# tensorlink-lab/tensorlink

Hardware: AMD Instinct MI355X
Metric: output tokens/sec (Qwen2.5-7B serving, PP sharded) (higher is better)
Workload: dtype bf16; 1 GPU; model=Qwen/Qwen2.5-7B-Instruct, global_batch=256, seq_len=512, parallelism=pp1, micro_batches=4

## Files before the change

### tensorlink_amd/models/dense.py

```python

from __future__ import annotations

import dataclasses

import math
from typing import List, Optional

import torch
import torch.nn as nn

from tensorlink_amd import ops
from tensorlink_amd.models.configs import ModelConfig


class KVCache:

    def __init__(self, n_layers: int, batch: int, max_seq: int, config,
                 device, dtype=torch.bfloat16):
        self.k = [torch.zeros(batch, config.num_key_value_heads, max_seq,
                              config.head_dim, device=device, dtype=dtype)
                  for _ in range(n_layers)]
        self.v = [torch.zeros_like(self.k[0]) for _ in range(n_layers)]
        self.seq_lens = torch.zeros(batch, device=device, dtype=torch.int32)
        self.max_seq = max_seq
        self.batch = batch

    def reset(self):
        self.seq_lens.zero_()

    def append(self, layer: int, k_new: torch.Tensor, v_new: torch.Tensor,
               positions: torch.Tensor):
        B, S_new, Hkv, D = k_new.shape
        idx = positions.to(self.k[layer].device, torch.long)
        idx = idx.view(B, 1, S_new, 1).expand(B, Hkv, S_new, D)
        self.k[layer].scatter_(2, idx, k_new.transpose(1, 2))
        self.v[layer].scatter_(2, idx, v_new.transpose(1, 2))

    def advance(self, n: int):
        self.seq_lens += n


class TLLinear(nn.Linear):

    def forward(self, x):
        return ops.linear(x, self.weight, self.bias)


def compute_inv_freq(config: ModelConfig) -> torch.Tensor:
    D = config.head_dim
    inv = 1.0 / (config.rope_theta ** (
        torch.arange(0, D, 2, dtype=torch.float32) / D))
    rs = config.rope_scaling
    if rs and rs.get("rope_type", rs.get("type")) == "llama3":
        factor = rs["factor"]
        lo, hi = rs["low_freq_factor"], rs["high_freq_factor"]
        orig = rs["original_max_position_embeddings"]
        wavelen = 2 * math.pi / inv
        smooth = (orig / wavelen - lo) / (hi - lo)
        smoothed = (1 - smooth) / factor * inv + smooth * inv
        inv = torch.where(wavelen > orig / lo, inv / factor, inv)
        mid = (wavelen <= orig / lo) & (wavelen >= orig / hi)
        inv = torch.where(mid, smoothed, inv)
    return inv


class Attention(nn.Module):
    def __init__(self, config: ModelConfig):
        super().__init__()
        self.config = config
        h, q, kv = config.hidden_size, config.q_size, config.kv_size
        bias = config.qkv_bias
        self.qkv_proj = TLLinear(h, q + 2 * kv, bias=bias)
        self.o_proj = TLLinear(q, h, bias=False)
        self.q_size, self.kv_size = q, kv
        self.n_heads = config.num_attention_heads
        self.n_kv = config.num_key_value_heads
        self.head_dim = config.head_dim
        self.scale = 1.0 / math.sqrt(self.head_dim)
        self.use_qk_norm = config.architecture == "qwen3"
        if self.use_qk_norm:
            self.q_norm = nn.Parameter(torch.ones(self.head_dim))
            self.k_norm = nn.Parameter(torch.ones(self.head_dim))
        self.register_buffer("inv_freq", compute_inv_freq(config),
                             persistent=False)

    def _split_qkv(self, qkv, B, S):
        q, k, v = qkv.split([self.q_size, self.kv_size, self.kv_size],
                            dim=-1)
        q = q.reshape(B, S, self.n_heads, self.head_dim)
        k = k.reshape(B, S, self.n_kv, self.head_dim)
        v = v.reshape(B, S, self.n_kv, self.head_dim)
        return q, k, v

    def forward(self, x: torch.Tensor, positions: torch.Tensor,
                kv_cache: Optional[KVCache] = None, layer_idx: int = 0,
                training: bool = False) -> torch.Tensor:
        B, S, H = x.shape
        eps = self.config.rms_norm_eps
        qkv = self.qkv_proj(x)
        flat_pos = positions.reshape(-1)

        if training or kv_cache is None:
            q, k, v = self._split_qkv(qkv, B, S)
            if self.use_qk_norm:
                q = ops.rmsnorm(q.contiguous(), self.q_norm.to(q.dtype), eps)
                k = ops.rmsnorm(k.contiguous(), self.k_norm.to(k.dtype), eps)
            if training:
                q2, k2 = ops.apply_rope(q.reshape(B * S, self.n_heads, -1),
                                        k.reshape(B * S, self.n_kv, -1),
                                        flat_pos, self.inv_freq)
                q = q2.view(B, S, self.n_heads, -1)
                k = k2.view(B, S, self.n_kv, -1)
                out = ops.attention_train(q, k, v, causal=True,
                                          scale=self.scale)
            else:
                q = q.contiguous()
                k = k.contiguous()
                ops.apply_rope_(q.view(B * S, self.n_heads, -1),
                                k.view(B * S, self.n_kv, -1), flat_pos,
                                self.inv_freq)
                out = ops.attention_prefill(q, k, v.contiguous(),
                                            causal=True, scale=self.scale)
            return self.o_proj(out.reshape(B, S, -1))

        table = getattr(kv_cache, "table", None)
        if self.use_qk_norm:
            q, k, v = self._split_qkv(qkv, B, S)
            q = ops.rmsnorm(q.contiguous(), self.q_norm.to(q.dtype), eps)
            k = ops.rmsnorm(k.contiguous(), self.k_norm.to(k.dtype), eps)
            qkv = torch.cat([q.reshape(B, S, -1), k.reshape(B, S, -1),
                             v.reshape(B, S, -1)], dim=-1)
        q = ops.rope_append_(qkv.reshape(B * S, -1), kv_cache.k[layer_idx],
                             kv_cache.v[layer_idx], flat_pos, self.inv_freq,
                             S, self.n_heads, self.n_kv, block_table=table)
        q = q.view(B, S, self.n_heads, self.head_dim)
        if S == 1:
            out = ops.attention_decode(
                q, kv_cache.k[layer_idx], kv_cache.v[layer_idx],
                kv_cache.seq_lens + 1, scale=self.scale, block_table=table)
        else:
            if B > 1:
                assert int(kv_cache.seq_lens.min()) == \
                    int(kv_cache.seq_lens.max()), \
                    "ragged cached prefill needs per-row q_off"
            off = int(kv_cache.seq_lens.max())
            kv_len = off + S
            if table is None:
                k_attn = kv_cache.k[layer_idx][:, :, :kv_len].permute(
                    0, 2, 1, 3).contiguous()
                v_attn = kv_cache.v[layer_idx][:, :, :kv_len].permute(
                    0, 2, 1, 3).contiguous()
            else:
                k_attn, v_attn = kv_cache.gather_contiguous(layer_idx, kv_len)
            out = ops.attention_prefill(q, k_attn, v_attn, causal=True,
                                        scale=self.scale, q_off=off)
        return self.o_proj(out.reshape(B, S, -1))


class MLP(nn.Module):
    def __init__(self, config: ModelConfig):
        super().__init__()
        h, i = config.hidden_size, config.intermediate_size
        self.inter = i
        self.gate_up_proj = TLLinear(h, 2 * i, bias=False)
        self.down_proj = TLLinear(i, h, bias=False)

    def forward(self, x):
        gu = self.gate_up_proj(x)
        if torch.is_grad_enabled() and gu.requires_grad:
            gate, up = gu.split([self.inter, self.inter], dim=-1)
            return self.down_proj(ops.swiglu(gate.contiguous(),
                                             up.contiguous()))
        return self.down_proj(ops.swiglu_fused(gu))


class MoEMLP(nn.Module):

    def __init__(self, config: ModelConfig):
        super().__init__()
        h, i = config.hidden_size, config.intermediate_size
        self.num_experts = config.num_local_experts
        self.top_k = config.num_experts_per_tok
        self.gate = nn.Linear(h, self.num_experts, bias=False)
        expert_cfg = (config if config.expert_intermediate_size == i
                      else dataclasses.replace(
                          config,
                          intermediate_size=config.expert_intermediate_size))
        self.experts = nn.ModuleList([MLP(expert_cfg)
                                      for _ in range(self.num_experts)])

    def _fused_kind(self):
        from tensorlink_amd.models.quant import Fp4Linear, Fp8Linear
        e0 = self.experts[0]
        if isinstance(e0.gate_up_proj, Fp8Linear):
            return "fp8"
        if isinstance(e0.gate_up_proj, Fp4Linear):
            for e in self.experts:
                for p in (e.gate_up_proj, e.down_proj):
                    if not (isinstance(p, Fp4Linear) and p.bias is None
                            and p.out_features % 64 == 0
                            and p.in_features % 128 == 0):
                        return None
            return "fp4"
        if isinstance(e0.gate_up_proj, nn.Linear) \
                and e0.gate_up_proj.bias is None:
            return "bf16"
        return None

    def _tables(self, dev, kind):
        wname = {"fp8": "weight_fp8", "fp4": "packed"}.get(kind, "weight")
        sname = {"fp8": "scale", "fp4": "exponents"}.get(kind)
        gus = [getattr(e.gate_up_proj, wname) for e in self.experts]
        key = (str(dev), kind, gus[0].data_ptr())
        if getattr(self, "_tbl_key", None) != key:
            downs = [getattr(e.down_proj, wname) for e in self.experts]

            def mk(ts):
                if kind == "fp4":
                    assert all(t.is_contiguous()
                               and t.data_ptr() % 16 == 0 for t in ts), \
                        "fp4 expert tensors must be contiguous and " \
                        "16-byte aligned"
                return torch.tensor([t.data_ptr() for t in ts],
                                    dtype=torch.int64, device=dev)
            self._gu_ptrs = mk(gus)
            self._down_ptrs = mk(downs)
            if sname is not None:
                self._gu_scales = mk([getattr(e.gate_up_proj, sname)
                                      for e in self.experts])
                self._down_scales = mk([getattr(e.down_proj, sname)
                                        for e in self.experts])
            else:
                self._gu_scales = self._down_scales = None
            self._tbl_key = key
        return (self._gu_ptrs, self._down_ptrs, self._gu_scales,
                self._down_scales)

    def _fused_forward(self, flat, rw, idx, kind=None):
        C = ops._require_ext()
        kind = kind if kind is not None else self._fused_kind()
        E, k = self.num_experts, self.top_k
        T, H = flat.shape
        P = T * k
        dev = flat.device
        gu_p, down_p, gu_s, down_s = self._tables(dev, kind)
        fi = idx.reshape(-1)
        order = fi.argsort(stable=True)
        counts = torch.zeros(E, device=dev, dtype=torch.long)
        counts.scatter_add_(0, fi, torch.ones_like(fi))
        seg = torch.zeros(E + 1, device=dev, dtype=torch.int32)
        seg[1:] = counts.cumsum(0)
        pair_tok = (order // k).to(torch.int32)
        Ie = self.experts[0].inter
        if kind == "fp4":
            gu = ops.mxfp4_moe_gemm(flat.contiguous(), pair_tok, seg, gu_p,
                                    gu_s, 2 * Ie)
            act = ops.swiglu_fused(gu)
            y_pairs = ops.mxfp4_moe_gemm(act, None, seg, down_p, down_s, H)
        else:
            fp8 = kind == "fp8"
            gu = C.moe_gemm(flat.contiguous(), pair_tok, seg, gu_p, gu_s,
                            2 * Ie, fp8)
            act = ops.swiglu_fused(gu)
            y_pairs = C.moe_gemm(act, None, seg, down_p, down_s, H, fp8)
        y_pairs = y_pairs * rw.reshape(-1)[order].unsqueeze(1)
        inv = torch.empty_like(order)
        inv[order] = torch.arange(P, device=dev, dtype=order.dtype)
        return y_pairs[inv].view(T, k, H).sum(1)

    def forward(self, x):
        B, S, H = x.shape
        flat = x.reshape(-1, H)
        weights, idx = ops.moe_topk_router(self.gate(flat), self.top_k)
        weights = weights.to(x.dtype)
        if (flat.is_cuda and flat.dtype == torch.bfloat16
                and not torch.is_grad_enabled() and ops.extension_loaded()):
            kind = self._fused_kind()
            if kind is not None:
                out = self._fused_forward(flat, weights, idx, kind)
                return out.reshape(B, S, H)
        out = torch.zeros_like(flat)
        for e in range(self.num_experts):
            mask = (idx == e)
            tok, slot = mask.nonzero(as_tuple=True)
            if tok.numel() == 0:
                continue
            out.index_add_(0, tok,
                           self.experts[e](flat[tok]) * weights[tok, slot, None])
        return out.reshape(B, S, H)


class DecoderLayer(nn.Module):
    def __init__(self, config: ModelConfig):
        super().__init__()
        self.config = config
        self.input_layernorm = nn.Parameter(torch.ones(config.hidden_size))
        self.post_attention_layernorm = nn.Parameter(
            torch.ones(config.hidden_size))
        self.self_attn = Attention(config)
        self.mlp = MoEMLP(config) if config.is_moe else MLP(config)

    def forward(self, hidden, positions, kv_cache=None, layer_idx=0,
                training=False):
        eps = self.config.rms_norm_eps
        w_in = self.input_layernorm.to(hidden.dtype)
        w_post = self.post_attention_layernorm.to(hidden.dtype)
        if training or not hidden.is_cuda:
            h = ops.rmsnorm(hidden, w_in, eps)
            hidden = hidden + self.self_attn(h, positions, kv_cache,
                                             layer_idx, training)
            h = ops.rmsnorm(hidden, w_post, eps)
            hidden = hidden + self.mlp(h)
            return hidden
        h = ops.rmsnorm(hidden, w_in, eps)
        attn_out = self.self_attn(h, positions, kv_cache, layer_idx, False)
        h, hidden = ops.rmsnorm_residual(attn_out, hidden, w_post, eps)
        return hidden + self.mlp(h)


class StageModel(nn.Module):

    def __init__(self, config: ModelConfig, layer_start: int, layer_end: int,
                 has_embedding: bool, has_head: bool):
        super().__init__()
        self.config = config
        self.layer_start = layer_start
        self.layer_end = layer_end
        self.has_embedding = has_embedding
        self.has_head = has_head
        if has_embedding:
            self.embed_tokens = nn.Embedding(config.vocab_size,
                                             config.hidden_size)
        self.layers = nn.ModuleList(
            [DecoderLayer(config) for _ in range(layer_end - layer_start)])
        if has_head:
            self.norm = nn.Parameter(torch.ones(config.hidden_size))
            if not (config.tie_word_embeddings and has_embedding):
                self.lm_head = TLLinear(config.hidden_size,
                                        config.vocab_size, bias=False)

    @property
    def num_layers(self):
        return len(self.layers)

    def make_kv_cache(self, batch: int, max_seq: int, device, dtype=None,
                      kv_mode: str = "contiguous"):
        if dtype is None:
            dtype = next(self.parameters()).dtype
        if kv_mode == "paged":
            from tensorlink_amd.models.paged import PagedKVCache
            return PagedKVCache(self.num_layers, batch, max_seq,
                                self.config, device, dtype)
        return KVCache(self.num_layers, batch, max_seq, self.config, device,
                       dtype)

    def embed(self, input_ids: torch.Tensor) -> torch.Tensor:
        w = self.embed_tokens.weight
        return self.embed_tokens(input_ids).to(w.dtype)

    def head(self, hidden: torch.Tensor) -> torch.Tensor:
        h = ops.rmsnorm(hidden, self.norm.to(hidden.dtype),
                        self.config.rms_norm_eps)
        if self.config.tie_word_embeddings and self.has_embedding:
            return h @ self.embed_tokens.weight.t()
        return self.lm_head(h)

    def forward(self, hidden_or_ids, positions, kv_cache: Optional[KVCache]
                = None, training: bool = False,
                return_logits: bool = True) -> torch.Tensor:
        if self.has_embedding and hidden_or_ids.dtype in (torch.int32,
                                                          torch.int64):
            hidden = self.embed(hidden_or_ids)
        else:
            hidden = hidden_or_ids
        ckpt = (training and getattr(self, "grad_checkpointing", False)
                and torch.is_grad_enabled())
        for i, layer in enumerate(self.layers):
            if ckpt:
                hidden = torch.utils.checkpoint.checkpoint(
                    layer, hidden, positions, kv_cache, i, training,
                    use_reentrant=False)
            else:
                hidden = layer(hidden, positions, kv_cache, i, training)
        if kv_cache is not None:
            kv_cache.advance(hidden.shape[1])
        if self.has_head and return_logits:
            return self.head(hidden)
        return hidden


def build_full_model(config: ModelConfig):
    cls = _stage_class(config)
    return cls(config, 0, config.num_hidden_layers, True, True)


def build_stage(config: ModelConfig, spec):
    cls = _stage_class(config)
    return cls(config, spec.layer_start, spec.layer_end,
               spec.has_embedding, spec.has_head)


def _stage_class(config: ModelConfig):
    if config.architecture == "gpt2":
        from tensorlink_amd.models.gpt2 import Gpt2StageModel
        return Gpt2StageModel
    if config.architecture == "neox":
        from tensorlink_amd.models.neox import NeoxStageModel
        return NeoxStageModel
    return StageModel
```

### tensorlink_amd/ops/__init__.py

```python

from __future__ import annotations

import math
from typing import Optional

import torch

from tensorlink_amd.ops import reference as ref

_C = None
_IMPORT_ERROR: Optional[BaseException] = None
try:
    from tensorlink_amd import _C
except Exception as e:
    _IMPORT_ERROR = e


def extension_loaded() -> bool:
    return _C is not None


def _require_ext():
    if _C is None:
        raise RuntimeError(
            "tensorlink_amd._C HIP extension is not built but a CUDA/HIP "
            "tensor reached the op layer. Build it in-tree with "
            "`PYTORCH_ROCM_ARCH=gfx950 python setup.py build_ext --inplace` "
            f"(import error: {_IMPORT_ERROR!r})")
    return _C


def _on_gpu(*tensors: torch.Tensor) -> bool:
    return any(t.is_cuda for t in tensors if isinstance(t, torch.Tensor))


class _RMSNormFn(torch.autograd.Function):
    @staticmethod
    def forward(ctx, x, weight, eps):
        C = _require_ext()
        need_grad = x.requires_grad or weight.requires_grad
        outs = C.rmsnorm_fwd(x.contiguous(), None, weight.contiguous(), eps,
                             need_grad)
        y = outs[0]
        if need_grad:
            ctx.save_for_backward(x, weight, outs[1])
        return y

    @staticmethod
    def backward(ctx, dy):
        C = _require_ext()
        x, weight, rstd = ctx.saved_tensors
        dx, dw = C.rmsnorm_bwd(dy.contiguous(), x.contiguous(),
                               weight.contiguous(), rstd)
        return dx, dw, None


def rmsnorm(x: torch.Tensor, weight: torch.Tensor, eps: float = 1e-6):
    if not _on_gpu(x):
        return ref.rmsnorm(x, weight, eps)
    if torch.is_grad_enabled() and (x.requires_grad or weight.requires_grad):
        return _RMSNormFn.apply(x, weight, eps)
    return _require_ext().rmsnorm_fwd(x.contiguous(), None,
                                      weight.contiguous(), eps, False)[0]


def rmsnorm_residual(x: torch.Tensor, residual: torch.Tensor,
                     weight: torch.Tensor, eps: float = 1e-6):
    if not _on_gpu(x):
        return ref.rmsnorm_residual(x, residual, weight, eps)
    outs = _require_ext().rmsnorm_fwd(x.contiguous(), residual.contiguous(),
                                      weight.contiguous(), eps, False)
    return outs[0], outs[1]


def apply_rope_(q: torch.Tensor, k: torch.Tensor, positions: torch.Tensor,
                inv_freq: torch.Tensor, sign: float = 1.0) -> None:
    if not _on_gpu(q):
        freqs = positions.float()[:, None] * inv_freq.float()[None, :]
        cos, sin = freqs.cos(), freqs.sin()
        qq, kk = ref.apply_rope(q.unsqueeze(0), k.unsqueeze(0), cos,
                                sin * sign)
        q.copy_(qq[0])
        k.copy_(kk[0])
        return
    _require_ext().rope_(q, k, positions.int(), inv_freq.float(), sign)


def rope_append_(qkv: torch.Tensor, k_cache: torch.Tensor,
                 v_cache: torch.Tensor, positions: torch.Tensor,
                 inv_freq: torch.Tensor, S: int, Hq: int, Hkv: int,
                 block_table: Optional[torch.Tensor] = None) -> torch.Tensor:
    if _on_gpu(qkv):
        return _require_ext().rope_append_(
            qkv.contiguous(), k_cache, v_cache, positions.int(),
            inv_freq.float(), S, Hq, Hkv,
            block_table.int() if block_table is not None else None)
    D = k_cache.shape[-1]
    T = qkv.numel() // qkv.shape[-1]
    q = qkv[..., :Hq * D].reshape(T, Hq, D).contiguous()
    k = qkv[..., Hq * D:(Hq + Hkv) * D].reshape(T, Hkv, D).contiguous()
    v = qkv[..., (Hq + Hkv) * D:].reshape(T, Hkv, D).contiguous()
    apply_rope_(q, k, positions, inv_freq)
    B = T // S
    pos = positions.view(B, S).long()
    kB = k.view(B, S, Hkv, D)
    vB = v.view(B, S, Hkv, D)
    if block_table is None:
        for b in range(B):
            k_cache[b, :, pos[b]] = kB[b].transpose(0, 1)
            v_cache[b, :, pos[b]] = vB[b].transpose(0, 1)
    else:
        for b in range(B):
            for s_i in range(S):
                p = int(pos[b, s_i])
                page = int(block_table[b, p // 128])
                k_cache[page, :, p % 128] = kB[b, s_i]
                v_cache[page, :, p % 128] = vB[b, s_i]
    return q


class _RopeFn(torch.autograd.Function):

    @staticmethod
    def forward(ctx, q, k, positions, inv_freq):
        q2, k2 = q.contiguous().clone(), k.contiguous().clone()
        apply_rope_(q2, k2, positions, inv_freq, 1.0)
        ctx.save_for_backward(positions, inv_freq)
        return q2, k2

    @staticmethod
    def backward(ctx, dq, dk):
        positions, inv_freq = ctx.saved_tensors
        dq2, dk2 = dq.contiguous().clone(), dk.contiguous().clone()
        apply_rope_(dq2, dk2, positions, inv_freq, -1.0)
        return dq2, dk2, None, None


def apply_rope(q, k, positions, inv_freq):
    return _RopeFn.apply(q, k, positions, inv_freq)


class _SwiGLUFn(torch.autograd.Function):
    @staticmethod
    def forward(ctx, gate, up):
        C = _require_ext()
        ctx.save_for_backward(gate, up)
        return C.swiglu_fwd(gate.contiguous(), up.contiguous())

    @staticmethod
    def backward(ctx, dout):
        C = _require_ext()
        gate, up = ctx.saved_tensors
        dg, du = C.swiglu_bwd(dout.contiguous(), gate.contiguous(),
                              up.contiguous())
        return dg, du


def swiglu(gate: torch.Tensor, up: torch.Tensor) -> torch.Tensor:
    if not _on_gpu(gate):
        return ref.swiglu(gate, up)
    if torch.is_grad_enabled() and (gate.requires_grad or up.requires_grad):
        return _SwiGLUFn.apply(gate, up)
    return _require_ext().swiglu_fwd(gate.contiguous(), up.contiguous())


def swiglu_fused(gate_up: torch.Tensor) -> torch.Tensor:
    if not _on_gpu(gate_up):
        I = gate_up.shape[-1] // 2
        return ref.swiglu(gate_up[..., :I], gate_up[..., I:])
    return _require_ext().swiglu_fused(gate_up.contiguous())


def attention_prefill(q, k, v, causal: bool = True,
                      scale: Optional[float] = None,
                      q_off: int = 0) -> torch.Tensor:
    scale = scale if scale is not None else 1.0 / math.sqrt(q.shape[-1])
    if not _on_gpu(q):
        return ref.attention_prefill(q, k, v, causal, scale, q_off)
    if (q.shape[1] >= 4096 and q_off == 0 and causal
            and q.shape[1] == k.shape[1]):
        out = torch.nn.functional.scaled_dot_product_attention(
            q.transpose(1, 2), k.transpose(1, 2), v.transpose(1, 2),
            is_causal=True, scale=scale, enable_gqa=True)
        return out.transpose(1, 2)
    return _require_ext().prefill_attn(q.contiguous(), k.contiguous(),
                                       v.contiguous(), scale, causal,
                                       q_off)


class _FlashAttnFn(torch.autograd.Function):

    @staticmethod
    def forward(ctx, q, k, v, causal, scale):
        C = _require_ext()
        out, lse = C.prefill_attn_lse(q.contiguous(), k.contiguous(),
                                      v.contiguous(), scale, causal)
        ctx.save_for_backward(q, k, v, out, lse)
        ctx.causal = causal
        ctx.scale = scale
        return out

    @staticmethod
    def backward(ctx, dout):
        C = _require_ext()
        q, k, v, out, lse = ctx.saved_tensors
        delta = (dout.float() * out.float()).sum(-1)
        delta = delta.permute(0, 2, 1).contiguous()
        dq, dk, dv = C.attn_bwd(q.contiguous(), k.contiguous(),
                                v.contiguous(), dout.contiguous(), lse,
                                delta, ctx.scale, ctx.causal)
        return dq, dk, dv, None, None


def attention_train(q, k, v, causal: bool = True,
                    scale: Optional[float] = None) -> torch.Tensor:
    B, S, Hq, D = q.shape
    Hkv = k.shape[2]
    if scale is None:
        scale = 1.0 / math.sqrt(D)
    if (q.is_cuda and q.dtype == torch.bfloat16 and _C is not None
            and D in (64, 128) and k.shape[1] == S):
        return _FlashAttnFn.apply(q, k, v, causal, scale)
    qt = q.transpose(1, 2)
    kt = k.transpose(1, 2)
    vt = v.transpose(1, 2)
    try:
        out = torch.nn.functional.scaled_dot_product_attention(
            qt, kt, vt, is_causal=causal, scale=scale, enable_gqa=True)
    except (TypeError, RuntimeError):
        rep = Hq // Hkv
        out = torch.nn.functional.scaled_dot_product_attention(
            qt, kt.repeat_interleave(rep, dim=1),
            vt.repeat_interleave(rep, dim=1), is_causal=causal, scale=scale)
    return out.transpose(1, 2)


def attention_decode(q, k_cache, v_cache, seq_lens,
                     scale: Optional[float] = None, n_split: int = 0,
                     block_table: Optional[torch.Tensor] = None
                     ) -> torch.Tensor:
    squeeze = q.dim() == 4
    if squeeze:
        q3 = q.squeeze(1)
    else:
        q3 = q
    scale = scale if scale is not None else 1.0 / math.sqrt(q3.shape[-1])
    if not _on_gpu(q3):
        if block_table is not None:
            B = q3.shape[0]
            L = int(seq_lens.max())
            np_ = (L + 127) // 128
            idx = block_table[:, :np_].long()
            kc = k_cache[idx].permute(0, 1, 3, 2, 4)
            vc = v_cache[idx].permute(0, 1, 3, 2, 4)
            kc = kc.reshape(B, np_ * 128, *kc.shape[3:])[:, :L]
            vc = vc.reshape(B, np_ * 128, *vc.shape[3:])[:, :L]
            out = ref.attention_decode(q3.unsqueeze(1), kc, vc, seq_lens,
                                       scale)
        else:
            out = ref.attention_decode(q3.unsqueeze(1),
                                       k_cache.permute(0, 2, 1, 3),
                                       v_cache.permute(0, 2, 1, 3),
                                       seq_lens, scale)
        return out if squeeze else out.squeeze(1)
    out = _require_ext().decode_attn(
        q3.contiguous(), k_cache, v_cache, seq_lens.int(), scale, n_split,
        block_table.int() if block_table is not None else None)
    return out.unsqueeze(1) if squeeze else out


import os as _os

GEMM_M_MAX = int(_os.environ.get("TL_GEMM_M_MAX", "512"))

gemm_dispatch_count = 0


_LIB_CLASSES = frozenset(
    c for c in _os.environ.get("TL_GEMM_LIB_CLASSES",
                               "gateup").split(",") if c)


def _gemm_class(N: int, K: int) -> str:
    if N >= 65536:
        return "wide"
    if N >= 16384:
        return "gateup"
    if K >= 8192:
        return "deepk"
    return "narrow"


def _use_tl_gemm(M: int, N: int, K: int) -> bool:
    return (K % 32 == 0 and N % 64 == 0 and M <= GEMM_M_MAX
            and _gemm_class(N, K) not in _LIB_CLASSES)


def linear(x: torch.Tensor, weight: torch.Tensor,
           bias: Optional[torch.Tensor] = None) -> torch.Tensor:
    global gemm_dispatch_count
    if (x.is_cuda and not torch.is_grad_enabled()
            and x.dtype == torch.bfloat16
            and not _os.environ.get("TL_NO_SKINNY")):
        K = x.shape[-1]
        M = x.numel() // K
        N = weight.shape[0]
        if _use_tl_gemm(M, N, K):
            gemm_dispatch_count += 1
            return _require_ext().skinny_gemm(
                x.contiguous(), weight,
                bias.to(torch.bfloat16) if bias is not None else None)
    return torch.nn.functional.linear(x, weight, bias)


mxfp4_dispatch_count = 0


def _use_mxfp4_gemm(M: int, N: int, K: int) -> bool:
    return (N > 0 and N % 64 == 0 and K > 0 and K % 128 == 0
            and 1 <= M <= min(GEMM_M_MAX, 512))


def mxfp4_linear(x: torch.Tensor, packed: torch.Tensor,
                 exponents: torch.Tensor,
                 bias: Optional[torch.Tensor] = None) -> torch.Tensor:
    global mxfp4_dispatch_count
    if not _on_gpu(x):
        return ref.mxfp4_linear(x, packed, exponents, bias)
    K = x.shape[-1]
    M = x.numel() // K if K else 0
    N = packed.shape[0]
    if (x.dtype == torch.bfloat16 and _C is not None
            and _use_mxfp4_gemm(M, N, K)):
        mxfp4_dispatch_count += 1
        return _C.mxfp4_gemm(
            x.contiguous(), packed.contiguous(), exponents.contiguous(),
            bias.to(torch.bfloat16).contiguous()
            if bias is not None else None)
    w = ref.dequantize_mxfp4(packed, exponents, dtype=torch.bfloat16)
    return torch.nn.functional.linear(
        x, w.to(x.dtype), bias.to(x.dtype) if bias is not None else None)


mxfp4_moe_dispatch_count = 0


def mxfp4_moe_gemm(x: torch.Tensor, tok_idx: Optional[torch.Tensor],
                   seg_off: torch.Tensor, p_ptrs: torch.Tensor,
                   e_ptrs: torch.Tensor, N: int) -> torch.Tensor:
    global mxfp4_moe_dispatch_count
    out = _require_ext().mxfp4_moe_gemm(x, tok_idx, seg_off, p_ptrs, e_ptrs,
                                        N)
    mxfp4_moe_dispatch_count += 1
    return out


def adamw_(param: torch.Tensor, grad: torch.Tensor, exp_avg: torch.Tensor,
           exp_avg_sq: torch.Tensor, *, lr: float, beta1: float = 0.9,
           beta2: float = 0.999, eps: float = 1e-8,
           weight_decay: float = 0.0, step: int = 1) -> None:
    if not _on_gpu(param):
        ref.adamw_step(param, grad, exp_avg, exp_avg_sq, lr=lr, beta1=beta1,
                       beta2=beta2, eps=eps, weight_decay=weight_decay,
                       step=step)
        return
    _require_ext().adamw_(param, grad.contiguous(), exp_avg, exp_avg_sq, lr,
                          beta1, beta2, eps, weight_decay, step)


def _splitmix64(x: int) -> int:
    x = (x + 0x9E3779B97F4A7C15) & (2 ** 64 - 1)
    x = ((x ^ (x >> 30)) * 0xBF58476D1CE4E5B9) & (2 ** 64 - 1)
    x = ((x ^ (x >> 27)) * 0x94D049BB133111EB) & (2 ** 64 - 1)
    return x ^ (x >> 31)


def request_seed(seed: int, step: int) -> int:
    return _splitmix64((seed & (2 ** 63 - 1)) ^ (step * 0xA24BAED4963EE407)) \
        & (2 ** 63 - 1)


def sample_tokens(logits: torch.Tensor, *, temps, top_ps, top_ks, pres,
                  freqs, counts: Optional[torch.Tensor] = None,
                  seeds: Optional[torch.Tensor] = None,
                  counter: Optional[torch.Tensor] = None,
                  seed_base: int = 0) -> torch.Tensor:
    C = _require_ext()
    return C.sample_tokens(logits.contiguous(), temps, top_ps, top_ks,
                           pres, freqs, counts, seeds, counter, seed_base)


def sample_token(logits, *, temperature=1.0, top_p=1.0, top_k=0,
                 generator=None, token_counts=None,
                 presence_penalty=0.0, frequency_penalty=0.0):
    return ref.sample_token(logits, temperature=temperature, top_p=top_p,
                            top_k=top_k, generator=generator,
                            token_counts=token_counts,
                            presence_penalty=presence_penalty,
                            frequency_penalty=frequency_penalty)


moe_topk_router = ref.moe_topk_router
causal_lm_loss = ref.causal_lm_loss
rope_cos_sin = ref.rope_cos_sin


chunked_causal_lm_loss = ref.chunked_causal_lm_loss
```

### tensorlink_amd/ops/csrc/bindings.cpp

```cpp

#include <torch/extension.h>

#include <c10/hip/HIPStream.h>
#include <hip/hip_runtime.h>

extern "C" {
void tl_rmsnorm_fwd(const void* x, const void* residual, const void* w,
                    void* y, void* r_out, void* rstd, int64_t N, int H,
                    float eps, hipStream_t stream);
void tl_rmsnorm_bwd(const void* dy, const void* x, const void* w,
                    const void* rstd, void* dx, void* dw, void* dw_partial,
                    int n_blocks, int64_t N, int H, hipStream_t stream);
void tl_rope(void* q, void* k, const void* positions, const void* inv_freq,
             int64_t T, int Hq, int Hkv, int D, float sign,
             hipStream_t stream);
void tl_swiglu_fwd(const void* gate, const void* up, void* out, int64_t n,
                   hipStream_t stream);
void tl_swiglu_bwd(const void* dout, const void* gate, const void* up,
                   void* dgate, void* dup, int64_t n, hipStream_t stream);
void tl_adamw(void* param, const void* grad, void* m, void* v, int64_t n,
              int is_bf16, float lr, double beta1, double beta2, float eps,
              float weight_decay, int step, hipStream_t stream);
void tl_decode_attn(const void* q, const void* k_cache, const void* v_cache,
                    const void* seq_lens, void* out, int B, int Hq, int Hkv,
                    int Smax, int D, float scale, hipStream_t stream);
void tl_prefill_attn(const void* q, const void* k, const void* v, void* out,
                     int B, int Sq, int Skv, int q_off, int Hq, int Hkv,
                     int D, float scale, int causal, hipStream_t stream);
void tl_rope_append(const void* qkv, void* q_out, void* k_cache,
                    void* v_cache, const void* positions,
                    const void* inv_freq, const void* block_table,
                    int64_t T, int row_stride, int S, int Hq, int Hkv,
                    int D, int Smax, int bt_stride, hipStream_t stream);
void tl_swiglu_fused(const void* gu, void* out, int64_t N, int I,
                     hipStream_t stream);
void tl_decode_attn_mfma(const void* q, const void* k_cache,
                         const void* v_cache, const void* seq_lens,
                         const void* block_table, void* out,
                         void* partial, void* partial_ml, int B, int Hq,
                         int Hkv, int Smax, int D, float scale, int n_split,
                         int bt_stride, int per_row, hipStream_t stream);
void tl_skinny_gemm(const void* x, const void* w, const void* bias,
                    void* out, void* partial, int M, int N, int K,
                    int n_split, hipStream_t stream);
void tl_gemm_tiled(const void* x, const void* w, const void* bias, void* out,
                   void* partial, int M, int N, int K, int n_split,
                   hipStream_t stream);
void tl_sample(const void* logits, const void* temps, const void* top_ps,
               const void* top_ks, const void* pres, const void* freqs,
               void* counts, const void* seeds, const void* ctr, void* out,
               uint64_t seed_base, int B, int V, hipStream_t stream);
void tl_bump_counter(void* ctr, hipStream_t stream);
void tl_moe_gemm(const void* x, const void* tok_idx, const void* seg_off,
                 const void* w_ptrs, const void* s_ptrs, void* out, int E,
                 int N, int K, int fp8, hipStream_t stream);
void tl_mxfp4_gemm(const void* x, const void* packed, const void* exps,
                   const void* bias, void* out, void* partial, int M, int N,
                   int K, int n_split, hipStream_t stream);
void tl_mxfp4_moe_gemm(const void* x, const void* tok_idx,
                       const void* seg_off, const void* p_ptrs,
                       const void* e_ptrs, void* out, void* partial, int T,
                       int P, int E, int N, int K, int n_split,
                       hipStream_t stream);
void tl_prefill_attn_lse(const void* q, const void* k, const void* v,
                         void* out, void* lse, int B, int Sq, int Skv,
                         int q_off, int Hq, int Hkv, int D, float scale,
                         int causal, hipStream_t stream);
void tl_attn_bwd(const void* q, const void* k, const void* v,
                 const void* dout, const void* lse, const void* delta,
                 void* dq, void* dk, void* dv, int B, int S, int Hq,
                 int Hkv, int D, float scale, int causal,
                 hipStream_t stream);
}

namespace {

hipStream_t cur_stream() {
  return c10::hip::getCurrentHIPStream().stream();
}

int tl_split_for_len(int L) {
  int ns = 1;
  while (ns < 16 && L > 1024 * ns) ns <<= 1;
  return ns;
}

#define CHECK_IN(t, d)                                              \
  TORCH_CHECK((t).is_cuda(), #t " must be on GPU");                 \
  TORCH_CHECK((t).is_contiguous(), #t " must be contiguous");       \
  TORCH_CHECK((t).scalar_type() == (d), #t " wrong dtype")

using torch::Tensor;

std::vector<Tensor> rmsnorm_fwd(Tensor x, c10::optional<Tensor> residual,
                                Tensor w, double eps, bool save_rstd) {
  CHECK_IN(x, torch::kBFloat16);
  CHECK_IN(w, torch::kBFloat16);
  const int H = x.size(-1);
  TORCH_CHECK(H % 8 == 0, "H must be divisible by 8");
  TORCH_CHECK(H <= 16384, "rmsnorm supports H <= 16384");
  const int64_t N = x.numel() / H;
  auto y = torch::empty_like(x);
  Tensor rstd, r_out;
  if (save_rstd) rstd = torch::empty({N}, x.options().dtype(torch::kFloat));
  const void* res_ptr = nullptr;
  void* rout_ptr = nullptr;
  if (residual.has_value()) {
    CHECK_IN(residual.value(), torch::kBFloat16);
    r_out = torch::empty_like(x);
    res_ptr = residual->data_ptr();
    rout_ptr = r_out.data_ptr();
  }
  tl_rmsnorm_fwd(x.data_ptr(), res_ptr, w.data_ptr(), y.data_ptr(), rout_ptr,
                 save_rstd ? rstd.data_ptr() : nullptr, N, H, (float)eps,
                 cur_stream());
  std::vector<Tensor> outs = {y};
  if (residual.has_value()) outs.push_back(r_out);
  if (save_rstd) outs.push_back(rstd);
  return outs;
}

std::vector<Tensor> rmsnorm_bwd(Tensor dy, Tensor x, Tensor w, Tensor rstd) {
  CHECK_IN(dy, torch::kBFloat16);
  CHECK_IN(x, torch::kBFloat16);
  CHECK_IN(w, torch::kBFloat16);
  CHECK_IN(rstd, torch::kFloat);
  const int H = x.size(-1);
  TORCH_CHECK(H % 8 == 0, "H must be divisible by 8");
  TORCH_CHECK(H <= 16384, "rmsnorm supports H <= 16384");
  const int64_t N = x.numel() / H;
  const int n_blocks = (int)std::min<int64_t>(N, 512);
  auto dx = torch::empty_like(x);
  auto dw = torch::empty_like(w);
  auto partial = torch::empty({n_blocks, (int64_t)H},
                              x.options().dtype(torch::kFloat));
  tl_rmsnorm_bwd(dy.data_ptr(), x.data_ptr(), w.data_ptr(), rstd.data_ptr(),
                 dx.data_ptr(), dw.data_ptr(), partial.data_ptr(), n_blocks,
                 N, H, cur_stream());
  return {dx, dw};
}

void rope_(Tensor q, Tensor k, Tensor positions, Tensor inv_freq,
           double sign) {
  CHECK_IN(q, torch::kBFloat16);
  CHECK_IN(k, torch::kBFloat16);
  CHECK_IN(positions, torch::kInt);
  CHECK_IN(inv_freq, torch::kFloat);
  const int D = q.size(-1);
  const int Hq = q.size(-2);
  const int Hkv = k.size(-2);
  const int64_t T = q.numel() / ((int64_t)Hq * D);
  TORCH_CHECK(k.numel() / ((int64_t)Hkv * D) == T, "q/k token mismatch");
  TORCH_CHECK(positions.numel() == T, "positions size mismatch");
  tl_rope(q.data_ptr(), k.data_ptr(), positions.data_ptr(),
          inv_freq.data_ptr(), T, Hq, Hkv, D, (float)sign, cur_stream());
}

Tensor swiglu_fwd(Tensor gate, Tensor up) {
  CHECK_IN(gate, torch::kBFloat16);
  CHECK_IN(up, torch::kBFloat16);
  TORCH_CHECK(gate.numel() % 8 == 0, "numel must be divisible by 8");
  auto out = torch::empty_like(gate);
  tl_swiglu_fwd(gate.data_ptr(), up.data_ptr(), out.data_ptr(), gate.numel(),
                cur_stream());
  return out;
}

std::vector<Tensor> swiglu_bwd(Tensor dout, Tensor gate, Tensor up) {
  CHECK_IN(dout, torch::kBFloat16);
  auto dg = torch::empty_like(gate);
  auto du = torch::empty_like(up);
  tl_swiglu_bwd(dout.data_ptr(), gate.data_ptr(), up.data_ptr(), dg.data_ptr(),
                du.data_ptr(), gate.numel(), cur_stream());
  return {dg, du};
}

void adamw_(Tensor param, Tensor grad, Tensor m, Tensor v, double lr,
            double beta1, double beta2, double eps, double weight_decay,
            int64_t step) {
  TORCH_CHECK(param.is_cuda() && param.is_contiguous());
  TORCH_CHECK(m.scalar_type() == torch::kFloat &&
              v.scalar_type() == torch::kFloat);
  TORCH_CHECK(grad.scalar_type() == param.scalar_type());
  const bool is_bf16 = param.scalar_type() == torch::kBFloat16;
  TORCH_CHECK(is_bf16 || param.scalar_type() == torch::kFloat);
  tl_adamw(param.data_ptr(), grad.data_ptr(), m.data_ptr(), v.data_ptr(),
           param.numel(), is_bf16 ? 1 : 0, (float)lr, beta1, beta2,
           (float)eps, (float)weight_decay, (int)step,
           cur_stream());
}

Tensor decode_attn(Tensor q, Tensor k_cache, Tensor v_cache, Tensor seq_lens,
                   double scale, int64_t n_split,
                   c10::optional<Tensor> block_table) {
  CHECK_IN(q, torch::kBFloat16);
  CHECK_IN(k_cache, torch::kBFloat16);
  CHECK_IN(v_cache, torch::kBFloat16);
  CHECK_IN(seq_lens, torch::kInt);
  const int B = q.size(0), Hq = q.size(1), D = q.size(2);
  const int Hkv = k_cache.size(1), Smax = k_cache.size(2);
  const int G = Hq / Hkv;
  const void* bt = nullptr;
  int bt_stride = 0;
  if (block_table.has_value()) {
    CHECK_IN(block_table.value(), torch::kInt);
    TORCH_CHECK(G <= 16, "paged decode requires GQA group <= 16");
    TORCH_CHECK(k_cache.size(2) == 128, "paged pool PAGE must be 128");
    bt = block_table->data_ptr();
    bt_stride = block_table->size(1);
  }
  TORCH_CHECK(D == 64 || D == 128, "head_dim must be 64 or 128");
  TORCH_CHECK(Hq % Hkv == 0, "GQA requires Hq % Hkv == 0");
  auto out = torch::empty_like(q);
  const bool legacy = (getenv("TL_DECODE_LEGACY") != nullptr || G > 16) &&
                      bt == nullptr;
  if (legacy) {
    tl_decode_attn(q.data_ptr(), k_cache.data_ptr(), v_cache.data_ptr(),
                   seq_lens.data_ptr(), out.data_ptr(), B, Hq, Hkv, Smax, D,
                   (float)scale, cur_stream());
    return out;
  }
  int per_row = 0;
  if (n_split <= 0) {
    per_row = 1;
    const int upper = bt ? bt_stride * 128 : Smax;
    n_split = tl_split_for_len(upper);
  }
  TORCH_CHECK(n_split <= 64, "n_split too large");
  Tensor partial, partial_ml;
  void *pp = nullptr, *pml = nullptr;
  if (n_split > 1) {
    partial = torch::empty({(int64_t)B * Hq * n_split * D},
                           q.options().dtype(torch::kFloat));
    partial_ml = torch::empty({(int64_t)B * Hq * n_split * 2},
                              q.options().dtype(torch::kFloat));
    pp = partial.data_ptr();
    pml = partial_ml.data_ptr();
  }
  tl_decode_attn_mfma(q.data_ptr(), k_cache.data_ptr(), v_cache.data_ptr(),
                      seq_lens.data_ptr(), bt, out.data_ptr(), pp, pml, B,
                      Hq, Hkv, Smax, D, (float)scale, (int)n_split,
                      bt_stride, per_row, cur_stream());
  return out;
}

Tensor prefill_attn(Tensor q, Tensor k, Tensor v, double scale, bool causal,
                    int64_t q_off) {
  CHECK_IN(q, torch::kBFloat16);
  CHECK_IN(k, torch::kBFloat16);
  CHECK_IN(v, torch::kBFloat16);
  const int B = q.size(0), Sq = q.size(1), Hq = q.size(2), D = q.size(3);
  const int Skv = k.size(1);
  const int Hkv = k.size(2);
  TORCH_CHECK(D == 64 || D == 128, "head_dim must be 64 or 128");
  TORCH_CHECK(q_off + Sq <= Skv || !causal, "q_off + Sq must fit Skv");
  auto out = torch::empty_like(q);
  tl_prefill_attn(q.data_ptr(), k.data_ptr(), v.data_ptr(), out.data_ptr(),
                  B, Sq, Skv, (int)q_off, Hq, Hkv, D, (float)scale,
                  causal ? 1 : 0, cur_stream());
  return out;
}

std::vector<Tensor> prefill_attn_lse(Tensor q, Tensor k, Tensor v,
                                     double scale, bool causal) {
  CHECK_IN(q, torch::kBFloat16);
  CHECK_IN(k, torch::kBFloat16);
  CHECK_IN(v, torch::kBFloat16);
  const int B = q.size(0), Sq = q.size(1), Hq = q.size(2), D = q.size(3);
  const int Skv = k.size(1);
  const int Hkv = k.size(2);
  TORCH_CHECK(D == 64 || D == 128, "head_dim must be 64 or 128");
  auto out = torch::empty_like(q);
  auto lse = torch::empty({B, Hq, Sq}, q.options().dtype(torch::kFloat));
  tl_prefill_attn_lse(q.data_ptr(), k.data_ptr(), v.data_ptr(),
                      out.data_ptr(), lse.data_ptr(), B, Sq, Skv, 0, Hq,
                      Hkv, D, (float)scale, causal ? 1 : 0, cur_stream());
  return {out, lse};
}

std::vector<Tensor> attn_bwd(Tensor q, Tensor k, Tensor v, Tensor dout,
                             Tensor lse, Tensor delta, double scale,
                             bool causal) {
  CHECK_IN(q, torch::kBFloat16);
  CHECK_IN(k, torch::kBFloat16);
  CHECK_IN(v, torch::kBFloat16);
  CHECK_IN(dout, torch::kBFloat16);
  CHECK_IN(lse, torch::kFloat);
  CHECK_IN(delta, torch::kFloat);
  const int B = q.size(0), S = q.size(1), Hq = q.size(2), D = q.size(3);
  const int Hkv = k.size(2);
  TORCH_CHECK(k.size(1) == S, "training attention needs Sq == Skv");
  TORCH_CHECK(D == 64 || D == 128, "head_dim must be 64 or 128");
  auto dq = torch::empty_like(q);
  auto dk = torch::empty_like(k);
  auto dv = torch::empty_like(v);
  tl_attn_bwd(q.data_ptr(), k.data_ptr(), v.data_ptr(), dout.data_ptr(),
              lse.data_ptr(), delta.data_ptr(), dq.data_ptr(),
              dk.data_ptr(), dv.data_ptr(), B, S, Hq, Hkv, D, (float)scale,
              causal ? 1 : 0, cur_stream());
  return {dq, dk, dv};
}

Tensor rope_append_(Tensor qkv, Tensor k_cache, Tensor v_cache,
                    Tensor positions, Tensor inv_freq, int64_t S,
                    int64_t Hq, int64_t Hkv,
                    c10::optional<Tensor> block_table) {
  CHECK_IN(qkv, torch::kBFloat16);
  CHECK_IN(k_cache, torch::kBFloat16);
  CHECK_IN(v_cache, torch::kBFloat16);
  CHECK_IN(positions, torch::kInt);
  CHECK_IN(inv_freq, torch::kFloat);
  const int D = k_cache.size(3);
  const int row_stride = qkv.size(-1);
  TORCH_CHECK(row_stride == (Hq + 2 * Hkv) * D, "qkv width mismatch");
  const int64_t T = qkv.numel() / row_stride;
  const int Smax = k_cache.size(2);
  TORCH_CHECK(T % S == 0, "T must be divisible by S");
  TORCH_CHECK(D % 16 == 0, "D must be divisible by 16");
  const void* bt = nullptr;
  int bt_stride = 0;
  if (block_table.has_value()) {
    CHECK_IN(block_table.value(), torch::kInt);
    TORCH_CHECK(k_cache.size(2) == 128, "paged pool PAGE must be 128");
    bt = block_table->data_ptr();
    bt_stride = block_table->size(1);
    TORCH_CHECK(block_table->size(0) * S == T, "table batch mismatch");
  } else {
    TORCH_CHECK(k_cache.size(0) * S == T, "cache batch mismatch");
  }
  auto q_out = torch::empty({T, Hq, (int64_t)D}, qkv.options());
  tl_rope_append(qkv.data_ptr(), q_out.data_ptr(), k_cache.data_ptr(),
                 v_cache.data_ptr(), positions.data_ptr(),
                 inv_freq.data_ptr(), bt, T, row_stride, (int)S, (int)Hq,
                 (int)Hkv, D, Smax, bt_stride, cur_stream());
  return q_out;
}

Tensor swiglu_fused(Tensor gu) {
  CHECK_IN(gu, torch::kBFloat16);
  const int64_t I2 = gu.size(-1);
  TORCH_CHECK(I2 % 16 == 0, "fused width must be divisible by 16");
  const int64_t I = I2 / 2;
  const int64_t N = gu.numel() / I2;
  auto sizes = gu.sizes().vec();
  sizes.back() = I;
  auto out = torch::empty(sizes, gu.options());
  tl_swiglu_fused(gu.data_ptr(), out.data_ptr(), N, (int)I, cur_stream());
  return out;
}

static int gemm_split_target() {
  static int t = [] {
    const char* e = getenv("TL_GEMM_SPLIT_TARGET");
    return e ? atoi(e) : 256;
  }();
  return t;
}

static int gemm_n_split(int N, int K) {
  if (N >= 65536) {
    int n_split = 1;
    while (((N + 255) / 256) * n_split < gemm_split_target() &&
           n_split < 16 && (K / 64) / (n_split * 2) >= 16)
      n_split <<= 1;
    return n_split;
  }
  int n_split = 1;
  while ((N / 64) * n_split < gemm_split_target() && n_split < 8 &&
         (K / 32) / (n_split * 2) >= 2)
    n_split <<= 1;
  return n_split;
}

Tensor skinny_gemm(Tensor x, Tensor w, c10::optional<Tensor> bias) {
  CHECK_IN(x, torch::kBFloat16);
  CHECK_IN(w, torch::kBFloat16);
  const int K = x.size(-1);
  const int64_t M = x.numel() / K;
  const int N = w.size(0);
  TORCH_CHECK(w.size(1) == K, "K mismatch");
  TORCH_CHECK(K % 32 == 0 && N % 64 == 0, "unsupported shape");
  auto sizes = x.sizes().vec();
  sizes.back() = N;
  auto out = torch::empty(sizes, x.options());
  const void* bp = nullptr;
  if (bias.has_value()) {
    CHECK_IN(bias.value(), torch::kBFloat16);
    bp = bias->data_ptr();
  }
  const int n_split = gemm_n_split(N, K);
  Tensor partial;
  void* pp = nullptr;
  if (n_split > 1) {
    partial = torch::empty({(int64_t)n_split * M * N},
                           x.options().dtype(torch::kFloat));
    pp = partial.data_ptr();
  }
  if (M <= 64)
    tl_skinny_gemm(x.data_ptr(), w.data_ptr(), bp, out.data_ptr(), pp,
                   (int)M, N, K, n_split, cur_stream());
  else
    tl_gemm_tiled(x.data_ptr(), w.data_ptr(), bp, out.data_ptr(), pp,
                  (int)M, N, K, n_split, cur_stream());
  return out;
}

static int mxfp4_split_for_blocks(int blocks, int K) {
  int n_split = 1;
  while (blocks * n_split < 256 && n_split < 8 &&
         (K / 128) / (n_split * 2) >= 2)
    n_split <<= 1;
  return n_split;
}

static int mxfp4_n_split(int N, int K) {
  return mxfp4_split_for_blocks(N / 64, K);
}

static int mxfp4_moe_n_split(int N, int K, int E) {
  return mxfp4_split_for_blocks((N / 64) * E, K);
}

int64_t mxfp4_n_split_py(int64_t N, int64_t K) {
  TORCH_CHECK(N > 0 && K > 0 && N % 64 == 0 && K % 128 == 0,
              "unsupported shape");
  return mxfp4_n_split((int)N, (int)K);
}

int64_t mxfp4_moe_n_split_py(int64_t N, int64_t K, int64_t E) {
  TORCH_CHECK(N > 0 && K > 0 && E > 0 && N % 64 == 0 && K % 128 == 0,
              "unsupported shape");
  return mxfp4_moe_n_split((int)N, (int)K, (int)E);
}

Tensor mxfp4_gemm(Tensor x, Tensor packed, Tensor exponents,
                  c10::optional<Tensor> bias) {
  CHECK_IN(x, torch::kBFloat16);
  CHECK_IN(packed, torch::kByte);
  CHECK_IN(exponents, torch::kChar);
  TORCH_CHECK(packed.dim() == 2 && exponents.dim() == 2,
              "packed / exponents must be 2-D");
  TORCH_CHECK(x.dim() >= 1, "x must have a K dimension");
  const int64_t K = x.size(-1);
  const int64_t N = packed.size(0);
  TORCH_CHECK(K > 0 && N > 0 && N % 64 == 0 && K % 128 == 0,
              "unsupported shape: need N % 64 == 0 and K % 128 == 0");
  TORCH_CHECK(packed.size(1) * 2 == K, "packed must be [N, K/2]");
  TORCH_CHECK(exponents.size(0) == N && exponents.size(1) * 32 == K,
              "exponents must be [N, K/32]");
  const int64_t M = x.numel() / K;
  TORCH_CHECK(M >= 1 && M <= 512, "mxfp4_gemm supports 1 <= M <= 512");
  TORCH_CHECK(packed.device() == x.device() &&
                  exponents.device() == x.device(),
              "operands must share a device");
  auto sizes = x.sizes().vec();
  sizes.back() = N;
  auto out = torch::empty(sizes, x.options());
  const void* bp = nullptr;
  if (bias.has_value()) {
    CHECK_IN(bias.value(), torch::kBFloat16);
    TORCH_CHECK(bias->numel() == N, "bias must be [N]");
    bp = bias->data_ptr();
  }
  const int n_split = mxfp4_n_split((int)N, (int)K);
  Tensor partial;
  void* pp = nullptr;
  if (n_split > 1) {
    partial = torch::empty({(int64_t)n_split * M * N},
                           x.options().dtype(torch::kFloat));
    pp = partial.data_ptr();
  }
  tl_mxfp4_gemm(x.data_ptr(), packed.data_ptr(), exponents.data_ptr(), bp,
                out.data_ptr(), pp, (int)M, (int)N, (int)K, n_split,
                cur_stream());
  return out;
}

Tensor sample_tokens(Tensor logits, Tensor temps, Tensor top_ps,
                     Tensor top_ks, Tensor pres, Tensor freqs,
                     c10::optional<Tensor> counts,
                     c10::optional<Tensor> seeds,
                     c10::optional<Tensor> counter, int64_t seed_base) {
  CHECK_IN(logits, torch::kBFloat16);
  CHECK_IN(temps, torch::kFloat);
  CHECK_IN(top_ps, torch::kFloat);
  CHECK_IN(top_ks, torch::kInt);
  CHECK_IN(pres, torch::kFloat);
  CHECK_IN(freqs, torch::kFloat);
  const int B = logits.size(0);
  const int V = logits.size(1);
  void* cnt = nullptr;
  if (counts.has_value()) {
    CHECK_IN(counts.value(), torch::kInt);
    TORCH_CHECK(counts->size(0) == B && counts->size(1) == V,
                "counts must be [B, V]");
    cnt = counts->data_ptr();
  }
  const void* sd = nullptr;
  if (seeds.has_value()) {
    CHECK_IN(seeds.value(), torch::kLong);
    sd = seeds->data_ptr();
  }
  const void* ct = nullptr;
  if (counter.has_value()) {
    CHECK_IN(counter.value(), torch::kLong);
    ct = counter->data_ptr();
  }
  auto out = torch::empty({B}, logits.options().dtype(torch::kLong));
  tl_sample(logits.data_ptr(), temps.data_ptr(), top_ps.data_ptr(),
            top_ks.data_ptr(), pres.data_ptr(), freqs.data_ptr(), cnt, sd,
            ct, out.data_ptr(), (uint64_t)seed_base, B, V, cur_stream());
  return out;
}

void bump_sample_counter(Tensor ctr) {
  CHECK_IN(ctr, torch::kLong);
  tl_bump_counter(ctr.data_ptr(), cur_stream());
}

Tensor moe_gemm(Tensor x, c10::optional<Tensor> tok_idx, Tensor seg_off,
                Tensor w_ptrs, c10::optional<Tensor> s_ptrs, int64_t N,
                bool fp8) {
  CHECK_IN(x, torch::kBFloat16);
  CHECK_IN(seg_off, torch::kInt);
  CHECK_IN(w_ptrs, torch::kLong);
  const int K = x.size(-1);
  TORCH_CHECK(K % 32 == 0 && N % 64 == 0, "unsupported MoE shape");
  const int E = w_ptrs.size(0);
  TORCH_CHECK(seg_off.size(0) == E + 1, "seg_off must be [E+1]");
  const void* ti = nullptr;
  int64_t P;
  if (tok_idx.has_value()) {
    CHECK_IN(tok_idx.value(), torch::kInt);
    ti = tok_idx->data_ptr();
    P = tok_idx->size(0);
  } else {
    P = x.size(0);
  }
  const void* sp = nullptr;
  if (fp8) {
    TORCH_CHECK(s_ptrs.has_value(), "fp8 needs scale pointers");
    CHECK_IN(s_ptrs.value(), torch::kLong);
    sp = s_ptrs->data_ptr();
  }
  auto out = torch::empty({P, N}, x.options());
  tl_moe_gemm(x.data_ptr(), ti, seg_off.data_ptr(), w_ptrs.data_ptr(), sp,
              out.data_ptr(), E, (int)N, K, fp8 ? 1 : 0, cur_stream());
  return out;
}

Tensor mxfp4_moe_gemm(Tensor x, c10::optional<Tensor> tok_idx,
                      Tensor seg_off, Tensor p_ptrs, Tensor e_ptrs,
                      int64_t N, int64_t n_split_override) {
  CHECK_IN(x, torch::kBFloat16);
  CHECK_IN(seg_off, torch::kInt);
  CHECK_IN(p_ptrs, torch::kLong);
  CHECK_IN(e_ptrs, torch::kLong);
  TORCH_CHECK(x.dim() == 2, "x must be [T, K]");
  const int64_t T = x.size(0);
  const int64_t K = x.size(1);
  TORCH_CHECK(K > 0 && N > 0 && N % 64 == 0 && K % 128 == 0,
              "unsupported shape: need N % 64 == 0 and K % 128 == 0");
  TORCH_CHECK(p_ptrs.dim() == 1 && e_ptrs.dim() == 1 &&
                  p_ptrs.size(0) == e_ptrs.size(0),
              "pointer tables must both be [E]");
  const int64_t E = p_ptrs.size(0);
  TORCH_CHECK(E >= 1 && E <= 65535, "need 1 <= E <= 65535");
  TORCH_CHECK(seg_off.dim() == 1 && seg_off.size(0) == E + 1,
              "seg_off must be [E+1]");
  TORCH_CHECK(seg_off.device() == x.device() &&
                  p_ptrs.device() == x.device() &&
                  e_ptrs.device() == x.device(),
              "operands must share a device");
  const void* ti = nullptr;
  int64_t P = T;
  if (tok_idx.has_value()) {
    CHECK_IN(tok_idx.value(), torch::kInt);
    TORCH_CHECK(tok_idx->dim() == 1, "tok_idx must be [P]");
    TORCH_CHECK(tok_idx->device() == x.device(),
                "operands must share a device");
    ti = tok_idx->data_ptr();
    P = tok_idx->size(0);
  }
  TORCH_CHECK(P * N < (int64_t)1 << 31 && T * K < (int64_t)1 << 40,
              "mxfp4_moe_gemm: call too large");
  auto out = torch::empty({P, N}, x.options());
  if (P == 0) return out;
  TORCH_CHECK(T >= 1, "x has no rows");
  const int n_split = n_split_override > 0
                          ? (int)n_split_override
                          : mxfp4_moe_n_split((int)N, (int)K, (int)E);
  TORCH_CHECK(n_split >= 1 && n_split <= 8, "bad split count");
  Tensor partial;
  void* pp = nullptr;
  if (n_split > 1) {
    partial = torch::empty({(int64_t)n_split * P * N},
                           x.options().dtype(torch::kFloat));
    pp = partial.data_ptr();
  }
  tl_mxfp4_moe_gemm(x.data_ptr(), ti, seg_off.data_ptr(), p_ptrs.data_ptr(),
                    e_ptrs.data_ptr(), out.data_ptr(), pp, (int)T, (int)P,
                    (int)E, (int)N, (int)K, n_split, cur_stream());
  return out;
}

}

PYBIND11_MODULE(TORCH_EXTENSION_NAME, mod) {
  mod.def("rope_append_", &rope_append_,
          "fused RoPE + KV-cache append from fused-QKV rows");
  mod.def("swiglu_fused", &swiglu_fused, "silu-mul on fused [.,2I] rows");
  mod.def("skinny_gemm", &skinny_gemm, "decode-M GEMM: x @ W^T + bias");
  mod.def("rmsnorm_fwd", &rmsnorm_fwd, "fused RMSNorm fwd (+residual)");
  mod.def("rmsnorm_bwd", &rmsnorm_bwd, "RMSNorm bwd");
  mod.def("rope_", &rope_, "in-place RoPE apply");
  mod.def("swiglu_fwd", &swiglu_fwd, "silu(gate)*up");
  mod.def("swiglu_bwd", &swiglu_bwd, "SwiGLU bwd");
  mod.def("adamw_", &adamw_, "fused AdamW step");
  mod.def("decode_attn", &decode_attn, "GQA decode attention over KV cache");
  mod.def("prefill_attn", &prefill_attn, "causal GQA prefill attention");
  mod.def("sample_tokens", &sample_tokens,
          "fused penalties/temperature/top-k/top-p sampling, one block/row");
  mod.def("bump_sample_counter", &bump_sample_counter,
          "advance the graph-safe sampling RNG counter");
  mod.def("moe_gemm", &moe_gemm,
          "grouped expert GEMM over expert-sorted pair rows");
  mod.def("mxfp4_gemm", &mxfp4_gemm,
          "weight-only MXFP4 GEMM: x @ dequant(packed, exponents)^T + bias");
  mod.def("mxfp4_n_split", &mxfp4_n_split_py,
          "split-K count of mxfp4_gemm for (N, K)");
  mod.def("mxfp4_moe_gemm", &mxfp4_moe_gemm,
          "grouped MXFP4 expert GEMM over expert-sorted pair rows",
          pybind11::arg("x"), pybind11::arg("tok_idx"),
          pybind11::arg("seg_off"), pybind11::arg("p_ptrs"),
          pybind11::arg("e_ptrs"), pybind11::arg("N"),
          pybind11::arg("n_split_override") = 0);
  mod.def("mxfp4_moe_n_split", &mxfp4_moe_n_split_py,
          "split-K count of mxfp4_moe_gemm for (N, K, E)");
  mod.def("prefill_attn_lse", &prefill_attn_lse,
          "causal GQA prefill attention returning (out, logsumexp)");
  mod.def("attn_bwd", &attn_bwd,
          "flash-attention backward: (dq, dk, dv) from saved lse/delta");
}
```

### tensorlink_amd/ops/csrc/common.hpp

```cpp
#pragma once

#include <hip/hip_runtime.h>
#include <hip/hip_bf16.h>
#include <hip/hip_fp16.h>
#include <cstdint>

#define WAVE_SIZE 64

#define DEVINLINE __device__ __forceinline__

using bf16 = __hip_bfloat16;
using bf16x2 = __hip_bfloat162;

struct alignas(16) bf16x8 {
  bf16 v[8];
};

union f32x4_u {
  float4 f4;
  float f[4];
};

DEVINLINE float bf2f(bf16 x) { return __bfloat162float(x); }
DEVINLINE bf16 f2bf(float x) { return __float2bfloat16(x); }

DEVINLINE float wave_reduce_sum(float x) {
#pragma unroll
  for (int off = 32; off > 0; off >>= 1) x += __shfl_xor(x, off, WAVE_SIZE);
  return x;
}

DEVINLINE float wave_reduce_max(float x) {
#pragma unroll
  for (int off = 32; off > 0; off >>= 1)
    x = fmaxf(x, __shfl_xor(x, off, WAVE_SIZE));
  return x;
}

template <int G>
DEVINLINE float group_reduce_sum(float x) {
#pragma unroll
  for (int off = G / 2; off > 0; off >>= 1) x += __shfl_xor(x, off, WAVE_SIZE);
  return x;
}

template <int NW>
DEVINLINE float block_reduce_sum(float x, float* lds) {
  const int lane = threadIdx.x & (WAVE_SIZE - 1);
  const int wave = threadIdx.x / WAVE_SIZE;
  x = wave_reduce_sum(x);
  if (lane == 0) lds[wave] = x;
  __syncthreads();
  float total = 0.f;
#pragma unroll
  for (int w = 0; w < NW; ++w) total += lds[w];
  return total;
}

__host__ __device__ inline int cdiv(int a, int b) { return (a + b - 1) / b; }

__host__ __device__ inline int tl_split_for_len(int L) {
  int ns = 1;
  while (ns < 16 && L > 1024 * ns) ns <<= 1;
  return ns;
}
__host__ __device__ inline int64_t cdiv64(int64_t a, int64_t b) {
  return (a + b - 1) / b;
}

typedef __bf16 tr_bf16x8 __attribute__((ext_vector_type(8)));

DEVINLINE tr_bf16x8 ds_read_tr16_frag(unsigned addr_bytes) {
  unsigned long long lo, hi;
  asm volatile(
      "ds_read_b64_tr_b16 %0, %2\n\t"
      "ds_read_b64_tr_b16 %1, %2 offset:128\n\t"
      "s_waitcnt lgkmcnt(0)"
      : "=v"(lo), "=v"(hi)
      : "v"(addr_bytes));
  union {
    struct { unsigned long long a, b; } u;
    tr_bf16x8 v;
  } cvt;
  cvt.u.a = lo;
  cvt.u.b = hi;
  return cvt.v;
}

DEVINLINE unsigned tr16_frag_addr(unsigned panel_base_bytes, int lane) {
  const int a = lane & 15, q = lane >> 4;
  return panel_base_bytes +
         (unsigned)(((q * 8 + (a >> 2)) * 16 + 4 * (a & 3)) * 2);
}

#define HIP_CHECK(expr)                                                     \
  do {                                                                      \
    hipError_t _e = (expr);                                                 \
    if (_e != hipSuccess) {                                                 \
      printf("HIP error %s at %s:%d\n", hipGetErrorString(_e), __FILE__,    \
             __LINE__);                                                     \
    }                                                                       \
  } while (0)
```

### tensorlink_amd/ops/csrc/decode_attn.hip

```cpp

#include "common.hpp"

namespace {

constexpr int BLOCK = 256;
constexpr int NWAVE = BLOCK / WAVE_SIZE;
constexpr int LPK = 8;
constexpr int KPW = WAVE_SIZE / LPK;

template <int D, int GMAX>
__global__ __launch_bounds__(BLOCK) void decode_attn_kernel(
    const bf16* __restrict__ q,
    const bf16* __restrict__ k_cache,
    const bf16* __restrict__ v_cache,
    const int* __restrict__ seq_lens,
    bf16* __restrict__ out,
    int Hq, int Hkv, int Smax, float scale) {
  constexpr int EPL = D / LPK;
  const int b = blockIdx.x;
  const int hkv = blockIdx.y;
  const int G = Hq / Hkv;
  const int g0 = blockIdx.z * GMAX;
  const int gq = min(GMAX, G - g0);
  const int h0 = hkv * G + g0;
  const int L = seq_lens[b];

  const int lane = threadIdx.x & (WAVE_SIZE - 1);
  const int wave = threadIdx.x / WAVE_SIZE;
  const int kg = lane / LPK;
  const int li = lane % LPK;

  __shared__ float q_lds[GMAX][D];
  __shared__ float red_m[NWAVE][GMAX];
  __shared__ float red_l[NWAVE][GMAX];
  __shared__ float red_o[NWAVE][GMAX][D];

  for (int i = threadIdx.x; i < gq * D; i += BLOCK) {
    const int g = i / D, d = i - g * D;
    q_lds[g][d] = bf2f(q[((int64_t)b * Hq + h0 + g) * D + d]);
  }
  __syncthreads();

  const bf16* kbase = k_cache + ((int64_t)b * Hkv + hkv) * Smax * D;
  const bf16* vbase = v_cache + ((int64_t)b * Hkv + hkv) * Smax * D;

  float m[GMAX], l[GMAX], acc[GMAX][EPL];
#pragma unroll
  for (int g = 0; g < GMAX; ++g) {
    m[g] = -1e30f;
    l[g] = 0.f;
#pragma unroll
    for (int e = 0; e < EPL; ++e) acc[g][e] = 0.f;
  }

  for (int k0 = wave * KPW; k0 < L; k0 += NWAVE * KPW) {
    const int key = k0 + kg;
    const bool valid = key < L;
    float kv_elems[EPL];
    {
      const bf16* kp = kbase + (int64_t)(valid ? key : 0) * D + li * EPL;
      const bf16x8* kp8 = reinterpret_cast<const bf16x8*>(kp);
#pragma unroll
      for (int c = 0; c < EPL / 8; ++c) {
        bf16x8 chunk = kp8[c];
#pragma unroll
        for (int j = 0; j < 8; ++j) kv_elems[c * 8 + j] = bf2f(chunk.v[j]);
      }
    }
    float p[GMAX];
#pragma unroll
    for (int g = 0; g < GMAX; ++g) {
      if (g >= gq) break;
      float dot = 0.f;
#pragma unroll
      for (int e = 0; e < EPL; ++e) dot += q_lds[g][li * EPL + e] * kv_elems[e];
      dot = group_reduce_sum<LPK>(dot);
      float score = valid ? dot * scale : -1e30f;
      const float tile_max = wave_reduce_max(score);
      const float m_new = fmaxf(m[g], tile_max);
      const float alpha = __expf(m[g] - m_new);
      p[g] = valid ? __expf(score - m_new) : 0.f;
      const float psum = wave_reduce_sum(li == 0 ? p[g] : 0.f);
      l[g] = l[g] * alpha + psum;
      m[g] = m_new;
#pragma unroll
      for (int e = 0; e < EPL; ++e) acc[g][e] *= alpha;
    }
    {
      const bf16* vp = vbase + (int64_t)(valid ? key : 0) * D + li * EPL;
      const bf16x8* vp8 = reinterpret_cast<const bf16x8*>(vp);
#pragma unroll
      for (int c = 0; c < EPL / 8; ++c) {
        bf16x8 chunk = vp8[c];
#pragma unroll
        for (int j = 0; j < 8; ++j) {
          const float ve = bf2f(chunk.v[j]);
#pragma unroll
          for (int g = 0; g < GMAX; ++g) {
            if (g >= gq) break;
            acc[g][c * 8 + j] += p[g] * ve;
          }
        }
      }
    }
  }

#pragma unroll
  for (int g = 0; g < GMAX; ++g) {
#pragma unroll
    for (int e = 0; e < EPL; ++e) {
#pragma unroll
      for (int off = LPK; off < WAVE_SIZE; off <<= 1)
        acc[g][e] += __shfl_xor(acc[g][e], off, WAVE_SIZE);
    }
  }

  if (kg == 0) {
#pragma unroll
    for (int g = 0; g < GMAX; ++g) {
      if (g < gq) {
#pragma unroll
        for (int e = 0; e < EPL; ++e) red_o[wave][g][li * EPL + e] = acc[g][e];
        if (li == 0) {
          red_m[wave][g] = m[g];
          red_l[wave][g] = l[g];
        }
      }
    }
  }
  __syncthreads();

  for (int i = threadIdx.x; i < gq * D; i += BLOCK) {
    const int g = i / D, d = i - g * D;
    float m_tot = -1e30f;
#pragma unroll
    for (int w = 0; w < NWAVE; ++w) m_tot = fmaxf(m_tot, red_m[w][g]);
    float l_tot = 0.f, o = 0.f;
#pragma unroll
    for (int w = 0; w < NWAVE; ++w) {
      const float f = __expf(red_m[w][g] - m_tot);
      l_tot += red_l[w][g] * f;
      o += red_o[w][g][d] * f;
    }
    out[((int64_t)b * Hq + h0 + g) * D + d] = f2bf(o / fmaxf(l_tot, 1e-30f));
  }
}

}

extern "C" {

void tl_decode_attn(const void* q, const void* k_cache, const void* v_cache,
                    const void* seq_lens, void* out, int B, int Hq, int Hkv,
                    int Smax, int D, float scale, hipStream_t stream) {
  const int G = Hq / Hkv;
  int gmax = G <= 2 ? 2 : 4;
  if (const char* e = getenv("TL_DECODE_GMAX")) gmax = atoi(e);
  dim3 grid(B, Hkv, (G + gmax - 1) / gmax), block(BLOCK);
#define LAUNCH(DD, GG)                                                     \
  hipLaunchKernelGGL((decode_attn_kernel<DD, GG>), grid, block, 0, stream, \
                     (const bf16*)q, (const bf16*)k_cache,                 \
                     (const bf16*)v_cache, (const int*)seq_lens,           \
                     (bf16*)out, Hq, Hkv, Smax, scale)
  if (D == 128) {
    if (gmax == 2) LAUNCH(128, 2);
    else if (gmax == 4) LAUNCH(128, 4);
    else LAUNCH(128, 8);
  } else if (D == 64) {
    if (gmax == 2) LAUNCH(64, 2);
    else if (gmax == 4) LAUNCH(64, 4);
    else LAUNCH(64, 8);
  }
#undef LAUNCH
}

}
```

### tensorlink_amd/ops/csrc/decode_attn_mfma.hip

```cpp

#include "common.hpp"

namespace {

constexpr int BLOCK = 256;
constexpr int NWAVE = 4;
constexpr int KT = 16;

using f32x4 = __attribute__((ext_vector_type(4))) float;
typedef __bf16 bf16x8_t __attribute__((ext_vector_type(8)));

template <int D, int SPLIT_MODE, int PAGED>
__global__ __launch_bounds__(BLOCK) void decode_attn_mfma_kernel(
    const bf16* __restrict__ q,
    const bf16* __restrict__ k_cache,
    const bf16* __restrict__ v_cache,
    const int* __restrict__ seq_lens,
    const int* __restrict__ block_table,
    bf16* __restrict__ out,
    float* __restrict__ partial,
    float* __restrict__ partial_ml,
    int Hq, int Hkv, int Smax, float scale, int n_split, int bt_stride,
    int per_row) {
  constexpr int KCH = D / 32;
  constexpr int NS = D / 16;
  const int b = blockIdx.x;
  const int hkv = blockIdx.y;
  const int split = blockIdx.z;
  const int G = Hq / Hkv;
  const int h0 = hkv * G;
  const int L = seq_lens[b];

  const int ns_row = per_row ? tl_split_for_len(L) : n_split;
  if (split >= ns_row) return;

  const int per_split = (L + ns_row - 1) / ns_row;
  const int k_begin = split * per_split;
  const int k_end = min(L, k_begin + per_split);

  const int lane = threadIdx.x & 63;
  const int wave = threadIdx.x >> 6;
  const int col = lane & 15;
  const int quad = lane >> 4;

  constexpr int PSTRIDE = 32 * 16 + 8;
  __shared__ bf16 v_pan[NWAVE * (D / 16) * PSTRIDE];
  __shared__ bf16 p_lds[NWAVE][16][32 + 8];
  __shared__ float red_m[NWAVE][16], red_l[NWAVE][16];
  __shared__ float red_o[NWAVE][16][D];

  for (int i = threadIdx.x; i < NWAVE * (D / 16); i += BLOCK) {
    for (int e = 0; e < 16 * 16; ++e)
      v_pan[i * PSTRIDE + 16 * 16 + e] = f2bf(0.f);
  }
  for (int i = threadIdx.x; i < NWAVE * 16; i += BLOCK) {
    for (int e = 16; e < 32; ++e) p_lds[i / 16][i % 16][e] = f2bf(0.f);
  }
  __syncthreads();

  const bf16* kbase = k_cache + ((int64_t)b * Hkv + hkv) * Smax * D;
  const bf16* vbase = v_cache + ((int64_t)b * Hkv + hkv) * Smax * D;

  bf16x8_t afrag[KCH];
  {
    const bool valid = col < G;
    const bf16* qrow = q + ((int64_t)b * Hq + h0 + (valid ? col : 0)) * D;
#pragma unroll
    for (int c = 0; c < KCH; ++c) {
      bf16x8_t f = *reinterpret_cast<const bf16x8_t*>(
          qrow + c * 32 + quad * 8);
      if (!valid)
#pragma unroll
        for (int j = 0; j < 8; ++j) f[j] = (__bf16)0.f;
      afrag[c] = f;
    }
  }

  float m_run[4], l_run[4];
  f32x4 oacc[NS];
#pragma unroll
  for (int r = 0; r < 4; ++r) { m_run[r] = -1e30f; l_run[r] = 0.f; }
#pragma unroll
  for (int n = 0; n < NS; ++n) oacc[n] = (f32x4){0.f, 0.f, 0.f, 0.f};

  for (int t0 = k_begin + wave * KT; t0 < k_end; t0 += NWAVE * KT) {
    const int key = t0 + col;
    const bool kv_ok = key < k_end;
    const int safe_key = kv_ok ? key : (k_end - 1);

    f32x4 sacc = (f32x4){0.f, 0.f, 0.f, 0.f};
    {
      const bf16 *krow, *vrow;
      if (PAGED) {
        const int page = block_table[b * bt_stride + (safe_key >> 7)];
        const int64_t off =
            (((int64_t)page * Hkv + hkv) * 128 + (safe_key & 127)) * D;
        krow = k_cache + off;
        vrow = v_cache + off;
      } else {
        krow = kbase + (int64_t)safe_key * D;
        vrow = vbase + (int64_t)safe_key * D;
      }
#pragma unroll
      for (int c = 0; c < KCH; ++c) {
        bf16x8_t kf = *reinterpret_cast<const bf16x8_t*>(
            krow + c * 32 + quad * 8);
        sacc = __builtin_amdgcn_mfma_f32_16x16x32_bf16(afrag[c], kf, sacc,
                                                       0, 0, 0);
        bf16x8_t vf = *reinterpret_cast<const bf16x8_t*>(
            vrow + c * 32 + quad * 8);
        const int d0 = c * 32 + quad * 8;
        const int pan = wave * (D / 16) + (d0 >> 4);
        *reinterpret_cast<bf16x8_t*>(
            &v_pan[pan * PSTRIDE + col * 16 + (d0 & 15)]) = vf;
      }
    }

    float p[4], row_max[4];
#pragma unroll
    for (int r = 0; r < 4; ++r) {
      sacc[r] = kv_ok ? sacc[r] * scale : -1e30f;
      row_max[r] = sacc[r];
    }
#pragma unroll
    for (int off = 1; off < 16; off <<= 1)
#pragma unroll
      for (int r = 0; r < 4; ++r)
        row_max[r] = fmaxf(row_max[r], __shfl_xor(row_max[r], off,
                                                  WAVE_SIZE));
    float m_new[4], alpha[4], psum[4];
#pragma unroll
    for (int r = 0; r < 4; ++r) {
      m_new[r] = fmaxf(m_run[r], row_max[r]);
      alpha[r] = __expf(m_run[r] - m_new[r]);
      p[r] = (kv_ok) ? __expf(sacc[r] - m_new[r]) : 0.f;
      psum[r] = p[r];
      m_run[r] = m_new[r];
    }
#pragma unroll
    for (int off = 1; off < 16; off <<= 1)
#pragma unroll
      for (int r = 0; r < 4; ++r)
        psum[r] += __shfl_xor(psum[r], off, WAVE_SIZE);
#pragma unroll
    for (int r = 0; r < 4; ++r) l_run[r] = l_run[r] * alpha[r] + psum[r];

#pragma unroll
    for (int r = 0; r < 4; ++r)
      p_lds[wave][quad * 4 + r][col] = f2bf(p[r]);
#pragma unroll
    for (int n = 0; n < NS; ++n)
#pragma unroll
      for (int r = 0; r < 4; ++r) oacc[n][r] *= alpha[r];

    bf16x8_t pa = *reinterpret_cast<const bf16x8_t*>(
        &p_lds[wave][col][quad * 8]);
#pragma unroll
    for (int n = 0; n < NS; ++n) {
      const unsigned pan_base = (unsigned)(uintptr_t)(
          &v_pan[(wave * (D / 16) + n) * PSTRIDE]);
      bf16x8_t vb = (bf16x8_t)ds_read_tr16_frag(
          tr16_frag_addr(pan_base, lane));
      oacc[n] = __builtin_amdgcn_mfma_f32_16x16x32_bf16(pa, vb, oacc[n],
                                                        0, 0, 0);
    }
  }

#pragma unroll
  for (int n = 0; n < NS; ++n)
#pragma unroll
    for (int r = 0; r < 4; ++r)
      red_o[wave][quad * 4 + r][n * 16 + col] = oacc[n][r];
  if (col == 0) {
#pragma unroll
    for (int r = 0; r < 4; ++r) {
      red_m[wave][quad * 4 + r] = m_run[r];
      red_l[wave][quad * 4 + r] = l_run[r];
    }
  }
  __syncthreads();

  const int g_count = min(G, 16);
  for (int i = threadIdx.x; i < g_count * D; i += BLOCK) {
    const int g = i / D, d = i - g * D;
    float m_tot = -1e30f;
#pragma unroll
    for (int w = 0; w < NWAVE; ++w) m_tot = fmaxf(m_tot, red_m[w][g]);
    float l_tot = 0.f, o = 0.f;
#pragma unroll
    for (int w = 0; w < NWAVE; ++w) {
      const float f = __expf(red_m[w][g] - m_tot);
      l_tot += red_l[w][g] * f;
      o += red_o[w][g][d] * f;
    }
    if (SPLIT_MODE) {
      const int64_t base = (((int64_t)b * Hq + h0 + g) * n_split + split);
      partial[base * D + d] = o;
      if (d == 0) {
        partial_ml[base * 2] = m_tot;
        partial_ml[base * 2 + 1] = l_tot;
      }
    } else {
      out[((int64_t)b * Hq + h0 + g) * D + d] =
          f2bf(o / fmaxf(l_tot, 1e-30f));
    }
  }
}

template <int D>
__global__ __launch_bounds__(128) void decode_attn_combine_kernel(
    const float* __restrict__ partial, const float* __restrict__ partial_ml,
    const int* __restrict__ seq_lens, bf16* __restrict__ out, int Hq,
    int n_split, int per_row) {
  const int bh = blockIdx.x;
  const int d = threadIdx.x;
  const int ns_row =
      per_row ? tl_split_for_len(seq_lens[bh / Hq]) : n_split;
  __shared__ float sm[64], sl[64];
  if (threadIdx.x < ns_row) {
    sm[threadIdx.x] = partial_ml[((int64_t)bh * n_split + threadIdx.x) * 2];
    sl[threadIdx.x] = partial_ml[((int64_t)bh * n_split + threadIdx.x) * 2 + 1];
  }
  __syncthreads();
  float m_tot = -1e30f;
  for (int s = 0; s < ns_row; ++s) m_tot = fmaxf(m_tot, sm[s]);
  float l_tot = 0.f, o = 0.f;
  for (int s = 0; s < ns_row; ++s) {
    const float f = __expf(sm[s] - m_tot);
    l_tot += sl[s] * f;
    o += partial[((int64_t)bh * n_split + s) * D + d] * f;
  }
  out[(int64_t)bh * D + d] = f2bf(o / fmaxf(l_tot, 1e-30f));
}

}

extern "C" {

void tl_decode_attn_mfma(const void* q, const void* k_cache,
                         const void* v_cache, const void* seq_lens,
                         const void* block_table, void* out,
                         void* partial, void* partial_ml, int B, int Hq,
                         int Hkv, int Smax, int D, float scale, int n_split,
                         int bt_stride, int per_row, hipStream_t stream) {
  dim3 grid(B, Hkv, n_split), block(BLOCK);
#define LAUNCH(DD, SM, PG)                                                   \
  hipLaunchKernelGGL((decode_attn_mfma_kernel<DD, SM, PG>), grid, block, 0,  \
                     stream, (const bf16*)q, (const bf16*)k_cache,           \
                     (const bf16*)v_cache, (const int*)seq_lens,             \
                     (const int*)block_table, (bf16*)out,                    \
                     (float*)partial, (float*)partial_ml, Hq, Hkv, Smax,     \
                     scale, n_split, bt_stride, per_row)
#define PICK(DD)                                                             \
  do {                                                                       \
    if (block_table) {                                                       \
      if (n_split == 1) LAUNCH(DD, 0, 1); else LAUNCH(DD, 1, 1);             \
    } else {                                                                 \
      if (n_split == 1) LAUNCH(DD, 0, 0); else LAUNCH(DD, 1, 0);             \
    }                                                                        \
  } while (0)
  if (D == 128) PICK(128);
  else if (D == 64) PICK(64);
#undef PICK
#undef LAUNCH
  if (n_split > 1) {
    dim3 cgrid(B * Hq), cblock(D);
    if (D == 128)
      hipLaunchKernelGGL((decode_attn_combine_kernel<128>), cgrid, cblock, 0,
                         stream, (const float*)partial,
                         (const float*)partial_ml, (const int*)seq_lens,
                         (bf16*)out, Hq, n_split, per_row);
    else
      hipLaunchKernelGGL((decode_attn_combine_kernel<64>), cgrid, cblock, 0,
                         stream, (const float*)partial,
                         (const float*)partial_ml, (const int*)seq_lens,
                         (bf16*)out, Hq, n_split, per_row);
  }
}

}
```

### tensorlink_amd/ops/csrc/gemm_tiled.hip

```cpp

#include "common.hpp"

namespace {

constexpr int BLOCK = 256;

using f32x4 = __attribute__((ext_vector_type(4))) float;
typedef __bf16 bf16x8_t __attribute__((ext_vector_type(8)));

template <int N>
DEVINLINE void waitcnt_vm() {
  asm volatile("s_waitcnt vmcnt(%0)" ::"n"(N) : "memory");
}

template <int MT, int HAS_BIAS, int SPLIT>
__global__ __launch_bounds__(BLOCK, 2) void gemm_tiled_kernel(
    const bf16* __restrict__ x,
    const bf16* __restrict__ w,
    const bf16* __restrict__ bias,
    bf16* __restrict__ out,
    float* __restrict__ partial,
    int M, int N, int K, int n_split) {
  constexpr int MPW = MT / 4;
  static_assert(MT % 4 == 0, "quadrant layout needs MT % 4 == 0");
  const int lane = threadIdx.x & 63;
  const int wave = threadIdx.x >> 6;
  const int col = lane & 15;
  const int quad = lane >> 4;
  const int m_base = blockIdx.z * (MT * 16);

  const int split = SPLIT ? blockIdx.y : 0;
  const int k_per = SPLIT ? ((K / 64 + n_split - 1) / n_split) * 64 : K;
  const int k_begin = split * k_per;
  const int k_end = min(K, k_begin + k_per);

  __shared__ bf16 lds[2][MT * 16 + 64][64];

  f32x4 acc[MT];
#pragma unroll
  for (int m = 0; m < MT; ++m) acc[m] = (f32x4){0.f, 0.f, 0.f, 0.f};

  constexpr int GPW = MT > 1 ? MT / 2 : 1;
  const int l8 = lane >> 3, c8 = lane & 7;

#define GT_GLDS_TILE(bufi, k0)                                              \
  if ((k0) < k_end) {                                                       \
    _Pragma("unroll") for (int g = 0; g < GPW; ++g) {                       \
      const int chunk = wave * GPW + g;                                     \
      if (chunk >= MT * 2) break;                   \
      const int row = chunk * 8 + l8;                                       \
      const int xr = min(m_base + row, M - 1);                              \
      const int kc = min((k0) + (c8 ^ (row & 7)) * 8, K - 8);               \
      auto gsrc = (const __attribute__((address_space(1))) void*)(          \
          x + (int64_t)xr * K + kc);                                        \
      auto ldst = (__attribute__((address_space(3))) void*)(                \
          &lds[bufi][chunk * 8][0]);                                        \
      __builtin_amdgcn_global_load_lds(gsrc, ldst, 16, 0, 0);               \
    }                                                                       \
    _Pragma("unroll") for (int g = 0; g < 2; ++g) {                         \
      const int wchunk = wave * 2 + g;                                      \
      const int wr = wchunk * 8 + l8;                                       \
      const int kc = min((k0) + (c8 ^ (wr & 7)) * 8, K - 8);                \
      auto gsrc = (const __attribute__((address_space(1))) void*)(          \
          w + ((int64_t)blockIdx.x * 64 + wr) * K + kc);                    \
      auto ldst = (__attribute__((address_space(3))) void*)(                \
          &lds[bufi][MT * 16 + wchunk * 8][0]);                             \
      __builtin_amdgcn_global_load_lds(gsrc, ldst, 16, 0, 0);               \
    }                                                                       \
  }

  constexpr int LPT = MT / 2 + 2;
  static_assert(MT == 8 || MT == 16, "LPT assumes wave-uniform chunks");
  GT_GLDS_TILE(0, k_begin);
  int buf = 0;
  for (int k0 = k_begin; k0 < k_end; k0 += 64) {
    if (k0 + 64 < k_end) {
      GT_GLDS_TILE(buf ^ 1, k0 + 64);
      waitcnt_vm<LPT>();
    } else {
      waitcnt_vm<0>();
    }
    __builtin_amdgcn_s_barrier();
    const int tile_k = min(64, k_end - k0);
#pragma unroll
    for (int kk = 0; kk < 2; ++kk) {
      if (kk * 32 < tile_k) {
        bf16x8_t bfrag[4], afrag[MPW];
#pragma unroll
        for (int nt = 0; nt < 4; ++nt) {
          const int wrow = nt * 16 + col;
          const int wslot = (kk * 4 + quad) ^ (wrow & 7);
          bfrag[nt] = *reinterpret_cast<const bf16x8_t*>(
              &lds[buf][MT * 16 + wrow][wslot * 8]);
        }
#pragma unroll
        for (int mt = 0; mt < MPW; ++mt) {
          const int row = wave * (MPW * 16) + mt * 16 + col;
          const int slot = (kk * 4 + quad) ^ (row & 7);
          afrag[mt] = *reinterpret_cast<const bf16x8_t*>(
              &lds[buf][row][slot * 8]);
        }
#pragma unroll
        for (int mt = 0; mt < MPW; ++mt)
#pragma unroll
          for (int nt = 0; nt < 4; ++nt)
            acc[mt * 4 + nt] = __builtin_amdgcn_mfma_f32_16x16x32_bf16(
                afrag[mt], bfrag[nt], acc[mt * 4 + nt], 0, 0, 0);
      }
    }
    asm volatile("s_waitcnt lgkmcnt(0)" ::: "memory");
    __builtin_amdgcn_s_barrier();
    buf ^= 1;
  }
#undef GT_GLDS_TILE

#pragma unroll
  for (int mt = 0; mt < MPW; ++mt) {
#pragma unroll
    for (int nt = 0; nt < 4; ++nt) {
      const int oc = blockIdx.x * 64 + nt * 16 + col;
      const float b = HAS_BIAS ? bf2f(bias[oc]) : 0.f;
#pragma unroll
      for (int r = 0; r < 4; ++r) {
        const int orow =
            m_base + wave * (MPW * 16) + mt * 16 + quad * 4 + r;
        if (orow < M) {
          if (SPLIT)
            partial[((int64_t)split * M + orow) * N + oc] =
                acc[mt * 4 + nt][r];
          else
            out[(int64_t)orow * N + oc] = f2bf(acc[mt * 4 + nt][r] + b);
        }
      }
    }
  }
}

template <int HAS_BIAS, int SPLIT>
__global__ __launch_bounds__(512, 1) void gemm_tiled_sq_kernel(
    const bf16* __restrict__ x,
    const bf16* __restrict__ w,
    const bf16* __restrict__ bias,
    bf16* __restrict__ out,
    float* __restrict__ partial,
    int M, int N, int K, int n_split) {
  const int lane = threadIdx.x & 63;
  const int wave = threadIdx.x >> 6;
  const int col = lane & 15;
  const int quad = lane >> 4;
  const int wm = wave >> 2;
  const int wn = wave & 3;
  const int m_base = blockIdx.z * 256;

  const int split = SPLIT ? blockIdx.y : 0;
  const int k_per = SPLIT ? ((K / 64 + n_split - 1) / n_split) * 64 : K;
  const int k_begin = split * k_per;
  const int k_end = min(K, k_begin + k_per);

  __shared__ bf16 lds[2][256 + 256][64];

  f32x4 acc[32];
#pragma unroll
  for (int m = 0; m < 32; ++m) acc[m] = (f32x4){0.f, 0.f, 0.f, 0.f};

  const int l8 = lane >> 3, c8 = lane & 7;

#define GS_GLDS_TILE(bufi, k0)                                              \
  if ((k0) < k_end) {                                                       \
    _Pragma("unroll") for (int g = 0; g < 4; ++g) {                         \
      const int chunk = wave * 4 + g;                                       \
      const int row = chunk * 8 + l8;                                       \
      const int xr = min(m_base + row, M - 1);                              \
      const int kc = min((k0) + (c8 ^ (row & 7)) * 8, K - 8);               \
      auto gsrc = (const __attribute__((address_space(1))) void*)(          \
          x + (int64_t)xr * K + kc);                                        \
      auto ldst = (__attribute__((address_space(3))) void*)(                \
          &lds[bufi][chunk * 8][0]);                                        \
      __builtin_amdgcn_global_load_lds(gsrc, ldst, 16, 0, 0);               \
    }                                                                       \
    _Pragma("unroll") for (int g = 0; g < 4; ++g) {                         \
      const int wchunk = wave * 4 + g;                                      \
      const int wr = wchunk * 8 + l8;                                       \
      const int gr = min((int)blockIdx.x * 256 + wr, N - 1);                \
      const int kc = min((k0) + (c8 ^ (wr & 7)) * 8, K - 8);                \
      auto gsrc = (const __attribute__((address_space(1))) void*)(          \
          w + (int64_t)gr * K + kc);                                        \
      auto ldst = (__attribute__((address_space(3))) void*)(                \
          &lds[bufi][256 + wchunk * 8][0]);                                 \
      __builtin_amdgcn_global_load_lds(gsrc, ldst, 16, 0, 0);               \
    }                                                                       \
  }

  GS_GLDS_TILE(0, k_begin);
  int buf = 0;
  for (int k0 = k_begin; k0 < k_end; k0 += 64) {
    if (k0 + 64 < k_end) {
      GS_GLDS_TILE(buf ^ 1, k0 + 64);
      waitcnt_vm<8>();
    } else {
      waitcnt_vm<0>();
    }
    __builtin_amdgcn_s_barrier();
    const int tile_k = min(64, k_end - k0);
#pragma unroll
    for (int kk = 0; kk < 2; ++kk) {
      if (kk * 32 < tile_k) {
        bf16x8_t bfrag[4], afrag[8];
#pragma unroll
        for (int nt = 0; nt < 4; ++nt) {
          const int wrow = wn * 64 + nt * 16 + col;
          const int wslot = (kk * 4 + quad) ^ (wrow & 7);
          bfrag[nt] = *reinterpret_cast<const bf16x8_t*>(
              &lds[buf][256 + wrow][wslot * 8]);
        }
#pragma unroll
        for (int mt = 0; mt < 8; ++mt) {
          const int row = wm * 128 + mt * 16 + col;
          const int slot = (kk * 4 + quad) ^ (row & 7);
          afrag[mt] = *reinterpret_cast<const bf16x8_t*>(
              &lds[buf][row][slot * 8]);
        }
#pragma unroll
        for (int mt = 0; mt < 8; ++mt)
#pragma unroll
          for (int nt = 0; nt < 4; ++nt)
            acc[mt * 4 + nt] = __builtin_amdgcn_mfma_f32_16x16x32_bf16(
                afrag[mt], bfrag[nt], acc[mt * 4 + nt], 0, 0, 0);
      }
    }
    asm volatile("s_waitcnt lgkmcnt(0)" ::: "memory");
    __builtin_amdgcn_s_barrier();
    buf ^= 1;
  }
#undef GS_GLDS_TILE

#pragma unroll
  for (int mt = 0; mt < 8; ++mt) {
#pragma unroll
    for (int nt = 0; nt < 4; ++nt) {
      const int oc = blockIdx.x * 256 + wn * 64 + nt * 16 + col;
      if (oc < N) {
        const float b = HAS_BIAS ? bf2f(bias[oc]) : 0.f;
#pragma unroll
        for (int r = 0; r < 4; ++r) {
          const int orow = m_base + wm * 128 + mt * 16 + quad * 4 + r;
          if (orow < M) {
            if (SPLIT)
              partial[((int64_t)split * M + orow) * N + oc] =
                  acc[mt * 4 + nt][r];
            else
              out[(int64_t)orow * N + oc] = f2bf(acc[mt * 4 + nt][r] + b);
          }
        }
      }
    }
  }
}

template <int HAS_BIAS>
__global__ void gemm_reduce_kernel(const float* __restrict__ partial,
                                   const bf16* __restrict__ bias,
                                   bf16* __restrict__ out, int64_t MN,
                                   int N, int n_split) {
  const int64_t i = (int64_t)blockIdx.x * blockDim.x + threadIdx.x;
  if (i >= MN) return;
  float acc = 0.f;
  for (int s = 0; s < n_split; ++s) acc += partial[s * MN + i];
  if (HAS_BIAS) acc += bf2f(bias[i % N]);
  out[i] = f2bf(acc);
}

}

extern "C" {

void tl_gemm_tiled(const void* x, const void* w, const void* bias, void* out,
                   void* partial, int M, int N, int K, int n_split,
                   hipStream_t stream) {
  const int m_tiles = (M + 15) / 16;
  const int split = n_split > 1 ? 1 : 0;
  if (N >= 65536) {
    dim3 wgrid(cdiv(N, 256), n_split, cdiv(M, 256)), wblock(512);
#define WDISPATCH(HB, SP)                                                   \
  hipLaunchKernelGGL((gemm_tiled_sq_kernel<HB, SP>), wgrid, wblock, 0,      \
                     stream, (const bf16*)x, (const bf16*)w,                \
                     (const bf16*)bias, (bf16*)out, (float*)partial, M, N,  \
                     K, n_split)
    if (split) WDISPATCH(0, 1);
    else if (bias) WDISPATCH(1, 0);
    else WDISPATCH(0, 0);
#undef WDISPATCH
  } else {
  const int MT = m_tiles <= 8 ? 8 : 16;
  const int n_mblk = cdiv(m_tiles, MT);
  dim3 grid(N / 64, n_split, n_mblk), block(BLOCK);
#define DISPATCH(MTV)                                                       \
  do {                                                                      \
    if (split) {                                                            \
      hipLaunchKernelGGL((gemm_tiled_kernel<MTV, 0, 1>), grid, block, 0,    \
                         stream, (const bf16*)x, (const bf16*)w, nullptr,   \
                         (bf16*)out, (float*)partial, M, N, K, n_split);    \
    } else if (bias) {                                                      \
      hipLaunchKernelGGL((gemm_tiled_kernel<MTV, 1, 0>), grid, block, 0,    \
                         stream, (const bf16*)x, (const bf16*)w,            \
                         (const bf16*)bias, (bf16*)out, nullptr, M, N, K,   \
                         1);                                                \
    } else {                                                                \
      hipLaunchKernelGGL((gemm_tiled_kernel<MTV, 0, 0>), grid, block, 0,    \
                         stream, (const bf16*)x, (const bf16*)w, nullptr,   \
                         (bf16*)out, nullptr, M, N, K, 1);                  \
    }                                                                       \
  } while (0)
  if (MT == 8) DISPATCH(8);
  else DISPATCH(16);
#undef DISPATCH
  }
  if (split) {
    const int64_t MN = (int64_t)M * N;
    dim3 rgrid((uint32_t)((MN + 255) / 256)), rblock(256);
    if (bias)
      hipLaunchKernelGGL((gemm_reduce_kernel<1>), rgrid, rblock, 0, stream,
                         (const float*)partial, (const bf16*)bias,
                         (bf16*)out, MN, N, n_split);
    else
      hipLaunchKernelGGL((gemm_reduce_kernel<0>), rgrid, rblock, 0, stream,
                         (const float*)partial, nullptr, (bf16*)out, MN, N,
                         n_split);
  }
}

}
```

### tensorlink_amd/ops/csrc/rmsnorm.hip

```cpp

#include "common.hpp"

namespace {

constexpr int BLOCK = 256;
constexpr int NW = BLOCK / WAVE_SIZE;

template <int ITERS, int RES>
__global__ __launch_bounds__(BLOCK) void rmsnorm_fwd_kernel(
    const bf16* __restrict__ x, const bf16* __restrict__ residual,
    const bf16* __restrict__ w, bf16* __restrict__ y, bf16* __restrict__ r_out,
    float* __restrict__ rstd_out, int H, float eps) {
  __shared__ float lds[NW];
  const int64_t row = blockIdx.x;
  const bf16* xrow = x + row * H;
  const bf16* rrow = RES ? residual + row * H : nullptr;

  float vals[ITERS][8];
  float sumsq = 0.f;
#pragma unroll
  for (int it = 0; it < ITERS; ++it) {
    const int base = (it * BLOCK + threadIdx.x) * 8;
    if (base < H) {
      bf16x8 vx = *reinterpret_cast<const bf16x8*>(xrow + base);
      if (RES) {
        bf16x8 vr = *reinterpret_cast<const bf16x8*>(rrow + base);
#pragma unroll
        for (int j = 0; j < 8; ++j) {
          float f = bf2f(vx.v[j]) + bf2f(vr.v[j]);
          vals[it][j] = f;
          sumsq += f * f;
        }
        bf16x8 out;
#pragma unroll
        for (int j = 0; j < 8; ++j) out.v[j] = f2bf(vals[it][j]);
        *reinterpret_cast<bf16x8*>(r_out + row * H + base) = out;
      } else {
#pragma unroll
        for (int j = 0; j < 8; ++j) {
          float f = bf2f(vx.v[j]);
          vals[it][j] = f;
          sumsq += f * f;
        }
      }
    } else {
#pragma unroll
      for (int j = 0; j < 8; ++j) vals[it][j] = 0.f;
    }
  }

  const float total = block_reduce_sum<NW>(sumsq, lds);
  const float rstd = rsqrtf(total / H + eps);
  if (threadIdx.x == 0 && rstd_out != nullptr) rstd_out[row] = rstd;

#pragma unroll
  for (int it = 0; it < ITERS; ++it) {
    const int base = (it * BLOCK + threadIdx.x) * 8;
    if (base < H) {
      bf16x8 vw = *reinterpret_cast<const bf16x8*>(w + base);
      bf16x8 out;
#pragma unroll
      for (int j = 0; j < 8; ++j)
        out.v[j] = f2bf(vals[it][j] * rstd * bf2f(vw.v[j]));
      *reinterpret_cast<bf16x8*>(y + row * H + base) = out;
    }
  }
}

template <int ITERS>
__global__ __launch_bounds__(BLOCK) void rmsnorm_bwd_kernel(
    const bf16* __restrict__ dy, const bf16* __restrict__ x,
    const bf16* __restrict__ w, const float* __restrict__ rstd,
    bf16* __restrict__ dx, float* __restrict__ dw_partial, int64_t N, int H) {
  __shared__ float lds[NW];
  float dw_acc[ITERS][8];
#pragma unroll
  for (int it = 0; it < ITERS; ++it)
#pragma unroll
    for (int j = 0; j < 8; ++j) dw_acc[it][j] = 0.f;

  for (int64_t row = blockIdx.x; row < N; row += gridDim.x) {
    const float rs = rstd[row];
    float xh[ITERS][8], g[ITERS][8];
    float dot = 0.f;
#pragma unroll
    for (int it = 0; it < ITERS; ++it) {
      const int base = (it * BLOCK + threadIdx.x) * 8;
      if (base < H) {
        bf16x8 vx = *reinterpret_cast<const bf16x8*>(x + row * H + base);
        bf16x8 vdy = *reinterpret_cast<const bf16x8*>(dy + row * H + base);
        bf16x8 vw = *reinterpret_cast<const bf16x8*>(w + base);
#pragma unroll
        for (int j = 0; j < 8; ++j) {
          float xhat = bf2f(vx.v[j]) * rs;
          float gv = bf2f(vdy.v[j]) * bf2f(vw.v[j]);
          xh[it][j] = xhat;
          g[it][j] = gv;
          dot += gv * xhat;
          dw_acc[it][j] += bf2f(vdy.v[j]) * xhat;
        }
      } else {
#pragma unroll
        for (int j = 0; j < 8; ++j) { xh[it][j] = 0.f; g[it][j] = 0.f; }
      }
    }
    const float mean_dot = block_reduce_sum<NW>(dot, lds) / H;
#pragma unroll
    for (int it = 0; it < ITERS; ++it) {
      const int base = (it * BLOCK + threadIdx.x) * 8;
      if (base < H) {
        bf16x8 out;
#pragma unroll
        for (int j = 0; j < 8; ++j)
          out.v[j] = f2bf((g[it][j] - xh[it][j] * mean_dot) * rs);
        *reinterpret_cast<bf16x8*>(dx + row * H + base) = out;
      }
    }
    __syncthreads();
  }

  float* slab = dw_partial + (int64_t)blockIdx.x * H;
#pragma unroll
  for (int it = 0; it < ITERS; ++it) {
    const int base = (it * BLOCK + threadIdx.x) * 8;
    if (base < H) {
#pragma unroll
      for (int j = 0; j < 8; ++j) slab[base + j] = dw_acc[it][j];
    }
  }
}

__global__ void reduce_partials_kernel(const float* __restrict__ partials,
                                       bf16* __restrict__ out, int P,
                                       int64_t H) {
  const int64_t i = (int64_t)blockIdx.x * blockDim.x + threadIdx.x;
  if (i >= H) return;
  float acc = 0.f;
  for (int p = 0; p < P; ++p) acc += partials[(int64_t)p * H + i];
  out[i] = f2bf(acc);
}

template <int RES>
void launch_fwd(const bf16* x, const bf16* res, const bf16* w, bf16* y,
                bf16* r_out, float* rstd, int64_t N, int H, float eps,
                hipStream_t s) {
  dim3 grid((uint32_t)N), block(BLOCK);
  const int iters = cdiv(H, BLOCK * 8);
#define CASE(I)                                                            \
  case I:                                                                  \
    hipLaunchKernelGGL((rmsnorm_fwd_kernel<I, RES>), grid, block, 0, s, x, \
                       res, w, y, r_out, rstd, H, eps);                    \
    break;
  switch (iters) {
    CASE(1) CASE(2) CASE(3) CASE(4) CASE(5) CASE(6) CASE(7) CASE(8)
    default: break;
  }
#undef CASE
}

}

extern "C" {

void tl_rmsnorm_fwd(const void* x, const void* residual, const void* w,
                    void* y, void* r_out, void* rstd, int64_t N, int H,
                    float eps, hipStream_t stream) {
  if (residual)
    launch_fwd<1>((const bf16*)x, (const bf16*)residual, (const bf16*)w,
                  (bf16*)y, (bf16*)r_out, (float*)rstd, N, H, eps, stream);
  else
    launch_fwd<0>((const bf16*)x, nullptr, (const bf16*)w, (bf16*)y, nullptr,
                  (float*)rstd, N, H, eps, stream);
}

void tl_rmsnorm_bwd(const void* dy, const void* x, const void* w,
                    const void* rstd, void* dx, void* dw, void* dw_partial,
                    int n_blocks, int64_t N, int H, hipStream_t stream) {
  const int iters = cdiv(H, BLOCK * 8);
  dim3 grid(n_blocks), block(BLOCK);
#define CASE(I)                                                               \
  case I:                                                                     \
    hipLaunchKernelGGL((rmsnorm_bwd_kernel<I>), grid, block, 0, stream,       \
                       (const bf16*)dy, (const bf16*)x, (const bf16*)w,       \
                       (const float*)rstd, (bf16*)dx, (float*)dw_partial, N,  \
                       H);                                                    \
    break;
  switch (iters) {
    CASE(1) CASE(2) CASE(3) CASE(4) CASE(5) CASE(6) CASE(7) CASE(8)
    default: break;
  }
#undef CASE
  dim3 rgrid(cdiv(H, 256)), rblock(256);
  hipLaunchKernelGGL(reduce_partials_kernel, rgrid, rblock, 0, stream,
                     (const float*)dw_partial, (bf16*)dw, n_blocks, H);
}

}
```

### tensorlink_amd/ops/csrc/rope_append.hip

```cpp

#include "common.hpp"

namespace {

constexpr int BLOCK = 256;

template <int PAGED>
__global__ __launch_bounds__(BLOCK) void rope_append_kernel(
    const bf16* __restrict__ qkv, bf16* __restrict__ q_out,
    bf16* __restrict__ k_cache, bf16* __restrict__ v_cache,
    const int* __restrict__ positions, const float* __restrict__ inv_freq,
    const int* __restrict__ block_table, int row_stride, int S, int Hq,
    int Hkv, int D, int Smax, int bt_stride) {
  const int64_t token = blockIdx.x;
  const int b = token / S;
  const int pos = positions[token];
  int64_t slot;
  if (PAGED) {
    const int page = block_table[b * bt_stride + (pos >> 7)];
    slot = ((int64_t)page * Hkv) * 128 + (pos & 127);
  } else {
    slot = ((int64_t)b * Hkv) * Smax + pos;
  }
  const int64_t head_stride = PAGED ? 128 : Smax;
  const int D2 = D / 2;
  const float fpos = (float)pos;
  const bf16* row = qkv + token * row_stride;
  const bf16* krow = row + Hq * D;
  const bf16* vrow = krow + Hkv * D;

  const int total = (Hq + Hkv) * D2;
  for (int idx = threadIdx.x; idx < total; idx += BLOCK) {
    const int h = idx / D2;
    const int d = idx - h * D2;
    float c, s;
    __sincosf(fpos * inv_freq[d], &s, &c);
    if (h < Hq) {
      const bf16* src = row + h * D;
      const float x1 = bf2f(src[d]);
      const float x2 = bf2f(src[d + D2]);
      bf16* dst = q_out + (token * Hq + h) * D;
      dst[d] = f2bf(x1 * c - x2 * s);
      dst[d + D2] = f2bf(x2 * c + x1 * s);
    } else {
      const int hk = h - Hq;
      const bf16* src = krow + hk * D;
      const float x1 = bf2f(src[d]);
      const float x2 = bf2f(src[d + D2]);
      bf16* kc = k_cache + (slot + hk * head_stride) * D;
      kc[d] = f2bf(x1 * c - x2 * s);
      kc[d + D2] = f2bf(x2 * c + x1 * s);
    }
  }
  const int vtotal = Hkv * D / 8;
  for (int idx = threadIdx.x; idx < vtotal; idx += BLOCK) {
    const int h = idx / (D / 8);
    const int d8 = idx - h * (D / 8);
    const bf16x8 val =
        *reinterpret_cast<const bf16x8*>(vrow + h * D + d8 * 8);
    reinterpret_cast<bf16x8*>(
        v_cache + (slot + h * head_stride) * D)[d8] = val;
  }
}

}

extern "C" {

void tl_rope_append(const void* qkv, void* q_out, void* k_cache,
                    void* v_cache, const void* positions,
                    const void* inv_freq, const void* block_table,
                    int64_t T, int row_stride, int S, int Hq, int Hkv,
                    int D, int Smax, int bt_stride, hipStream_t stream) {
  dim3 grid((uint32_t)T), block(BLOCK);
  if (block_table)
    hipLaunchKernelGGL((rope_append_kernel<1>), grid, block, 0, stream,
                       (const bf16*)qkv, (bf16*)q_out, (bf16*)k_cache,
                       (bf16*)v_cache, (const int*)positions,
                       (const float*)inv_freq, (const int*)block_table,
                       row_stride, S, Hq, Hkv, D, Smax, bt_stride);
  else
    hipLaunchKernelGGL((rope_append_kernel<0>), grid, block, 0, stream,
                       (const bf16*)qkv, (bf16*)q_out, (bf16*)k_cache,
                       (bf16*)v_cache, (const int*)positions,
                       (const float*)inv_freq, nullptr, row_stride, S, Hq,
                       Hkv, D, Smax, bt_stride);
}

}
```

### tensorlink_amd/ops/csrc/skinny_gemm.hip

```cpp

#include "common.hpp"

namespace {

constexpr int BLOCK = 256;

using f32x4 = __attribute__((ext_vector_type(4))) float;
typedef __bf16 bf16x8_t __attribute__((ext_vector_type(8)));

template <int MT, int HAS_BIAS, int SPLIT>
__global__ __launch_bounds__(BLOCK, 2) void skinny_gemm_kernel(
    const bf16* __restrict__ x,
    const bf16* __restrict__ w,
    const bf16* __restrict__ bias,
    bf16* __restrict__ out,
    float* __restrict__ partial,
    int M, int N, int K, int n_split) {
  const int lane = threadIdx.x & 63;
  const int wave = threadIdx.x >> 6;
  const int col = lane & 15;
  const int quad = lane >> 4;
  const int oc = blockIdx.x * 64 + wave * 16 + col;

  const int m_tiles = (M + 15) / 16;
  const int split = SPLIT ? blockIdx.y : 0;
  const int k_per = SPLIT ? ((K / 64 + n_split - 1) / n_split) * 64 : K;
  const int k_begin = split * k_per;
  const int k_end = min(K, k_begin + k_per);

  __shared__ bf16 x_lds[2][MT * 16][64];

  f32x4 acc[MT];
#pragma unroll
  for (int m = 0; m < MT; ++m) acc[m] = (f32x4){0.f, 0.f, 0.f, 0.f};

  const bf16* wrow = w + (int64_t)oc * K;

  constexpr int GPW = MT > 1 ? MT / 2 : 1;
  const int l8 = lane >> 3, c8 = lane & 7;

#define SG_GLDS_TILE(bufi, k0)                                              \
  if ((k0) < K) {                                                           \
    _Pragma("unroll") for (int g = 0; g < GPW; ++g) {                       \
      const int chunk = wave * GPW + g;          \
      if (chunk >= MT * 2) break;   \
      const int row = chunk * 8 + l8;                                       \
      const int xr = min(row, M - 1);                                       \
      const int kc = min((k0) + (c8 ^ (row & 7)) * 8, K - 8);               \
      auto gsrc = (const __attribute__((address_space(1))) void*)(          \
          x + (int64_t)xr * K + kc);                                        \
      auto ldst = (__attribute__((address_space(3))) void*)(                \
          &x_lds[bufi][chunk * 8][0]);                                      \
      __builtin_amdgcn_global_load_lds(gsrc, ldst, 16, 0, 0);               \
    }                                                                       \
  }

  SG_GLDS_TILE(0, k_begin);
  int buf = 0;
  for (int k0 = k_begin; k0 < k_end; k0 += 64) {
    __syncthreads();
    if (k0 + 64 < k_end)
      SG_GLDS_TILE(buf ^ 1, k0 + 64);
    const int tile_k = min(64, k_end - k0);
#pragma unroll
    for (int kk = 0; kk < 2; ++kk) {
      if (kk * 32 < tile_k) {
        bf16x8_t bfrag = *reinterpret_cast<const bf16x8_t*>(
            wrow + k0 + kk * 32 + quad * 8);
#pragma unroll
        for (int m = 0; m < MT; ++m) {
          const int row = m * 16 + col;
          const int slot = (kk * 4 + quad) ^ (row & 7);
          bf16x8_t afrag = *reinterpret_cast<const bf16x8_t*>(
              &x_lds[buf][row][slot * 8]);
          acc[m] = __builtin_amdgcn_mfma_f32_16x16x32_bf16(
              afrag, bfrag, acc[m], 0, 0, 0);
        }
      }
    }
    buf ^= 1;
  }
#undef SG_GLDS_TILE

  const float b = HAS_BIAS ? bf2f(bias[oc]) : 0.f;
#pragma unroll
  for (int m = 0; m < MT; ++m) {
#pragma unroll
    for (int r = 0; r < 4; ++r) {
      const int orow = m * 16 + quad * 4 + r;
      if (orow < M) {
        if (SPLIT)
          partial[((int64_t)split * M + orow) * N + oc] = acc[m][r];
        else
          out[(int64_t)orow * N + oc] = f2bf(acc[m][r] + b);
      }
    }
  }
}

template <int HAS_BIAS>
__global__ void skinny_reduce_kernel(const float* __restrict__ partial,
                                     const bf16* __restrict__ bias,
                                     bf16* __restrict__ out, int64_t MN,
                                     int N, int n_split) {
  const int64_t i = (int64_t)blockIdx.x * blockDim.x + threadIdx.x;
  if (i >= MN) return;
  float acc = 0.f;
  for (int s = 0; s < n_split; ++s) acc += partial[s * MN + i];
  if (HAS_BIAS) acc += bf2f(bias[i % N]);
  out[i] = f2bf(acc);
}

}

extern "C" {

void tl_skinny_gemm(const void* x, const void* w, const void* bias,
                    void* out, void* partial, int M, int N, int K,
                    int n_split, hipStream_t stream) {
  const int m_tiles = (M + 15) / 16;
  const int split = n_split > 1 ? 1 : 0;
  dim3 grid(N / 64, n_split), block(BLOCK);
#define DISPATCH(MT)                                                        \
  do {                                                                      \
    if (split) {                                                            \
      hipLaunchKernelGGL((skinny_gemm_kernel<MT, 0, 1>), grid, block, 0,    \
                         stream, (const bf16*)x, (const bf16*)w, nullptr,   \
                         (bf16*)out, (float*)partial, M, N, K, n_split);    \
    } else if (bias) {                                                      \
      hipLaunchKernelGGL((skinny_gemm_kernel<MT, 1, 0>), grid, block, 0,    \
                         stream, (const bf16*)x, (const bf16*)w,            \
                         (const bf16*)bias, (bf16*)out, nullptr, M, N, K,   \
                         1);                                                \
    } else {                                                                \
      hipLaunchKernelGGL((skinny_gemm_kernel<MT, 0, 0>), grid, block, 0,    \
                         stream, (const bf16*)x, (const bf16*)w, nullptr,   \
                         (bf16*)out, nullptr, M, N, K, 1);                  \
    }                                                                       \
  } while (0)
  if (m_tiles <= 1) DISPATCH(1);
  else if (m_tiles <= 2) DISPATCH(2);
  else if (m_tiles <= 4) DISPATCH(4);
  else if (m_tiles <= 8) DISPATCH(8);
  else DISPATCH(16);
#undef DISPATCH
  if (split) {
    const int64_t MN = (int64_t)M * N;
    dim3 rgrid((uint32_t)((MN + 255) / 256)), rblock(256);
    if (bias)
      hipLaunchKernelGGL((skinny_reduce_kernel<1>), rgrid, rblock, 0, stream,
                         (const float*)partial, (const bf16*)bias,
                         (bf16*)out, MN, N, n_split);
    else
      hipLaunchKernelGGL((skinny_reduce_kernel<0>), rgrid, rblock, 0, stream,
                         (const float*)partial, nullptr, (bf16*)out, MN, N,
                         n_split);
  }
}

}
```

Before: 13320 tokens/s.

## Fuse split-K GEMM reductions into rope-append and residual-add rmsnorm for decode

Adds a decode fusion path in which split-K skinny GEMM outputs stay as fp32 partials. They are summed inside the consumers: rope_append for QKV with bias, and a new add_rmsnorm kernel for o_proj and down_proj that also carries the residual across layers. This removes the separate reduce kernel launches and the bf16 round-trip of projection outputs. Attention decode also takes len_add so the seq_lens+1 tensor op is dropped. The risk is extra fp32 partial traffic into consumers, plus rounding-order differences.

```diff
diff --git a/tensorlink_amd/models/dense.py b/tensorlink_amd/models/dense.py
--- a/tensorlink_amd/models/dense.py
+++ b/tensorlink_amd/models/dense.py
@@ -44,6 +44,12 @@
 
     def forward(self, x):
         return ops.linear(x, self.weight, self.bias)
+
+
+def _project(mod: nn.Module, x: torch.Tensor, allow_bias: bool = False):
+    if type(mod) is TLLinear and (allow_bias or mod.bias is None):
+        return ops.linear_partials(x, mod.weight, mod.bias)
+    return mod(x)
 
 
 def compute_inv_freq(config: ModelConfig) -> torch.Tensor:
@@ -94,10 +100,14 @@
 
     def forward(self, x: torch.Tensor, positions: torch.Tensor,
                 kv_cache: Optional[KVCache] = None, layer_idx: int = 0,
-                training: bool = False) -> torch.Tensor:
+                training: bool = False, fuse: bool = False):
         B, S, H = x.shape
         eps = self.config.rms_norm_eps
-        qkv = self.qkv_proj(x)
+        fuse = fuse and kv_cache is not None and not training
+        if fuse and not self.use_qk_norm:
+            qkv = _project(self.qkv_proj, x, allow_bias=True)
+        else:
+            qkv = self.qkv_proj(x)
         flat_pos = positions.reshape(-1)
 
         if training or kv_cache is None:
@@ -130,11 +140,18 @@
             k = ops.rmsnorm(k.contiguous(), self.k_norm.to(k.dtype), eps)
             qkv = torch.cat([q.reshape(B, S, -1), k.reshape(B, S, -1),
                              v.reshape(B, S, -1)], dim=-1)
-        q = ops.rope_append_(qkv.reshape(B * S, -1), kv_cache.k[layer_idx],
+        if not isinstance(qkv, ops.Partials):
+            qkv = qkv.reshape(B * S, -1)
+        q = ops.rope_append_(qkv, kv_cache.k[layer_idx],
                              kv_cache.v[layer_idx], flat_pos, self.inv_freq,
                              S, self.n_heads, self.n_kv, block_table=table)
         q = q.view(B, S, self.n_heads, self.head_dim)
-        if S == 1:
+        if S == 1 and fuse:
+            out = ops.attention_decode(
+                q, kv_cache.k[layer_idx], kv_cache.v[layer_idx],
+                kv_cache.seq_lens, scale=self.scale, block_table=table,
+                len_add=1)
+        elif S == 1:
             out = ops.attention_decode(
                 q, kv_cache.k[layer_idx], kv_cache.v[layer_idx],
                 kv_cache.seq_lens + 1, scale=self.scale, block_table=table)
@@ -154,6 +171,8 @@
                 k_attn, v_attn = kv_cache.gather_contiguous(layer_idx, kv_len)
             out = ops.attention_prefill(q, k_attn, v_attn, causal=True,
                                         scale=self.scale, q_off=off)
+        if fuse:
+            return _project(self.o_proj, out.reshape(B, S, -1))
         return self.o_proj(out.reshape(B, S, -1))
 
 
@@ -165,12 +184,14 @@
         self.gate_up_proj = TLLinear(h, 2 * i, bias=False)
         self.down_proj = TLLinear(i, h, bias=False)
 
-    def forward(self, x):
+    def forward(self, x, fuse: bool = False):
         gu = self.gate_up_proj(x)
         if torch.is_grad_enabled() and gu.requires_grad:
             gate, up = gu.split([self.inter, self.inter], dim=-1)
             return self.down_proj(ops.swiglu(gate.contiguous(),
                                              up.contiguous()))
+        if fuse:
+            return _project(self.down_proj, ops.swiglu_fused(gu))
         return self.down_proj(ops.swiglu_fused(gu))
 
 
@@ -317,6 +338,23 @@
         h, hidden = ops.rmsnorm_residual(attn_out, hidden, w_post, eps)
         return hidden + self.mlp(h)
 
+    def forward_carry(self, residual, pending, positions, kv_cache=None,
+                      layer_idx=0):
+        eps = self.config.rms_norm_eps
+        w_in = self.input_layernorm.to(residual.dtype)
+        w_post = self.post_attention_layernorm.to(residual.dtype)
+        if pending is None:
+            h = ops.rmsnorm(residual, w_in, eps)
+        else:
+            h, residual = ops.add_rmsnorm(pending, residual, w_in, eps,
+                                          rounded=True)
+        attn_out = self.self_attn(h, positions, kv_cache, layer_idx, False,
+                                  fuse=True)
+        h, residual = ops.add_rmsnorm(attn_out, residual, w_post, eps)
+        if type(self.mlp) is MLP:
+            return residual, self.mlp(h, fuse=True)
+        return residual, self.mlp(h)
+
 
 class StageModel(nn.Module):
 
@@ -358,9 +396,14 @@
         w = self.embed_tokens.weight
         return self.embed_tokens(input_ids).to(w.dtype)
 
-    def head(self, hidden: torch.Tensor) -> torch.Tensor:
-        h = ops.rmsnorm(hidden, self.norm.to(hidden.dtype),
-                        self.config.rms_norm_eps)
+    def head(self, hidden: torch.Tensor, pending=None) -> torch.Tensor:
+        if pending is None:
+            h = ops.rmsnorm(hidden, self.norm.to(hidden.dtype),
+                            self.config.rms_norm_eps)
+        else:
+            h, _ = ops.add_rmsnorm(pending, hidden,
+                                   self.norm.to(hidden.dtype),
+                                   self.config.rms_norm_eps, rounded=True)
         if self.config.tie_word_embeddings and self.has_embedding:
             return h @ self.embed_tokens.weight.t()
         return self.lm_head(h)
@@ -375,6 +418,16 @@
             hidden = hidden_or_ids
         ckpt = (training and getattr(self, "grad_checkpointing", False)
                 and torch.is_grad_enabled())
+        if not training and ops.decode_fusion_enabled() and len(self.layers):
+            pending = None
+            for i, layer in enumerate(self.layers):
+                hidden, pending = layer.forward_carry(hidden, pending,
+                                                      positions, kv_cache, i)
+            if kv_cache is not None:
+                kv_cache.advance(hidden.shape[1])
+            if self.has_head and return_logits:
+                return self.head(hidden, pending)
+            return ops.add_residual(pending, hidden)
         for i, layer in enumerate(self.layers):
             if ckpt:
                 hidden = torch.utils.checkpoint.checkpoint(
diff --git a/tensorlink_amd/ops/__init__.py b/tensorlink_amd/ops/__init__.py
--- a/tensorlink_amd/ops/__init__.py
+++ b/tensorlink_amd/ops/__init__.py
@@ -71,6 +71,58 @@
     outs = _require_ext().rmsnorm_fwd(x.contiguous(), residual.contiguous(),
                                       weight.contiguous(), eps, False)
     return outs[0], outs[1]
+
+
+class Partials:
+
+    __slots__ = ("data", "bias")
+
+    def __init__(self, data: torch.Tensor, bias=None):
+        self.data = data
+        self.bias = bias
+
+    @property
+    def n_split(self) -> int:
+        return self.data.shape[0]
+
+    def materialize(self) -> torch.Tensor:
+        acc = torch.zeros_like(self.data[0])
+        for s in range(self.data.shape[0]):
+            acc = acc + self.data[s]
+        if self.bias is not None:
+            acc = acc + self.bias.float()
+        return acc.to(torch.bfloat16)
+
+
+def add_rmsnorm(x, residual: torch.Tensor, weight: torch.Tensor,
+                eps: float = 1e-6, rounded: bool = False):
+    part = isinstance(x, Partials)
+    if not _on_gpu(residual):
+        xt = x.materialize() if part else x
+        r = residual + xt
+        return ref.rmsnorm(r, weight, eps), r
+    if part:
+        assert x.bias is None, "add_rmsnorm takes bias-free partials"
+        xt = x.data
+    else:
+        xt = x.contiguous()
+    y, r = _require_ext().rmsnorm_add_fwd(
+        xt, residual.contiguous(), weight.contiguous(), eps,
+        2 if rounded else 1)
+    return y, r
+
+
+def add_residual(x, residual: torch.Tensor) -> torch.Tensor:
+    part = isinstance(x, Partials)
+    if not _on_gpu(residual):
+        return residual + (x.materialize() if part else x)
+    if part:
+        assert x.bias is None, "add_residual takes bias-free partials"
+        xt = x.data
+    else:
+        xt = x.contiguous()
+    return _require_ext().rmsnorm_add_fwd(xt, residual.contiguous(), None,
+                                          0.0, 3)[0]
 
 
 def apply_rope_(q: torch.Tensor, k: torch.Tensor, positions: torch.Tensor,
@@ -86,15 +138,24 @@
     _require_ext().rope_(q, k, positions.int(), inv_freq.float(), sign)
 
 
-def rope_append_(qkv: torch.Tensor, k_cache: torch.Tensor,
+def rope_append_(qkv, k_cache: torch.Tensor,
                  v_cache: torch.Tensor, positions: torch.Tensor,
                  inv_freq: torch.Tensor, S: int, Hq: int, Hkv: int,
                  block_table: Optional[torch.Tensor] = None) -> torch.Tensor:
-    if _on_gpu(qkv):
+    part = isinstance(qkv, Partials)
+    if _on_gpu(k_cache):
+        if inv_freq.dtype not in (torch.float32, torch.bfloat16):
+            inv_freq = inv_freq.float()
+        bt = block_table.int() if block_table is not None else None
+        if part:
+            return _require_ext().rope_append_(
+                qkv.data, k_cache, v_cache, positions.int(),
+                inv_freq.contiguous(), S, Hq, Hkv, bt, qkv.bias)
         return _require_ext().rope_append_(
             qkv.contiguous(), k_cache, v_cache, positions.int(),
-            inv_freq.float(), S, Hq, Hkv,
-            block_table.int() if block_table is not None else None)
+            inv_freq.contiguous(), S, Hq, Hkv, bt, None)
+    if part:
+        qkv = qkv.materialize()
     D = k_cache.shape[-1]
     T = qkv.numel() // qkv.shape[-1]
     q = qkv[..., :Hq * D].reshape(T, Hq, D).contiguous()
@@ -237,8 +298,8 @@
 
 def attention_decode(q, k_cache, v_cache, seq_lens,
                      scale: Optional[float] = None, n_split: int = 0,
-                     block_table: Optional[torch.Tensor] = None
-                     ) -> torch.Tensor:
+                     block_table: Optional[torch.Tensor] = None,
+                     len_add: int = 0) -> torch.Tensor:
     squeeze = q.dim() == 4
     if squeeze:
         q3 = q.squeeze(1)
@@ -246,6 +307,8 @@
         q3 = q
     scale = scale if scale is not None else 1.0 / math.sqrt(q3.shape[-1])
     if not _on_gpu(q3):
+        if len_add:
+            seq_lens = seq_lens + len_add
         if block_table is not None:
             B = q3.shape[0]
             L = int(seq_lens.max())
@@ -265,7 +328,7 @@
         return out if squeeze else out.squeeze(1)
     out = _require_ext().decode_attn(
         q3.contiguous(), k_cache, v_cache, seq_lens.int(), scale, n_split,
-        block_table.int() if block_table is not None else None)
+        block_table.int() if block_table is not None else None, len_add)
     return out.unsqueeze(1) if squeeze else out
 
 
@@ -311,6 +374,30 @@
                 x.contiguous(), weight,
                 bias.to(torch.bfloat16) if bias is not None else None)
     return torch.nn.functional.linear(x, weight, bias)
+
+
+def decode_fusion_enabled() -> bool:
+    return not _os.environ.get("TL_NO_DECODE_FUSION")
+
+
+def linear_partials(x: torch.Tensor, weight: torch.Tensor,
+                    bias: Optional[torch.Tensor] = None):
+    global gemm_dispatch_count
+    if (x.is_cuda and not torch.is_grad_enabled()
+            and x.dtype == torch.bfloat16
+            and not _os.environ.get("TL_NO_SKINNY")):
+        K = x.shape[-1]
+        M = x.numel() // K
+        N = weight.shape[0]
+        if _use_tl_gemm(M, N, K):
+            gemm_dispatch_count += 1
+            b = bias.to(torch.bfloat16) if bias is not None else None
+            out = _require_ext().skinny_gemm_partials(x.contiguous(),
+                                                      weight, b)
+            if out.dtype == torch.float32:
+                return Partials(out, b)
+            return out
+    return linear(x, weight, bias)
 
 
 mxfp4_dispatch_count = 0
diff --git a/tensorlink_amd/ops/csrc/bindings.cpp b/tensorlink_amd/ops/csrc/bindings.cpp
--- a/tensorlink_amd/ops/csrc/bindings.cpp
+++ b/tensorlink_amd/ops/csrc/bindings.cpp
@@ -8,6 +8,9 @@
 void tl_rmsnorm_fwd(const void* x, const void* residual, const void* w,
                     void* y, void* r_out, void* rstd, int64_t N, int H,
                     float eps, hipStream_t stream);
+void tl_rmsnorm_add_fwd(const void* x, const void* residual, const void* w,
+                        void* y, void* r_out, int64_t N, int H, float eps,
+                        int n_split, int mode, hipStream_t stream);
 void tl_rmsnorm_bwd(const void* dy, const void* x, const void* w,
                     const void* rstd, void* dx, void* dw, void* dw_partial,
                     int n_blocks, int64_t N, int H, hipStream_t stream);
@@ -23,15 +26,17 @@
               float weight_decay, int step, hipStream_t stream);
 void tl_decode_attn(const void* q, const void* k_cache, const void* v_cache,
                     const void* seq_lens, void* out, int B, int Hq, int Hkv,
-                    int Smax, int D, float scale, hipStream_t stream);
+                    int Smax, int D, float scale, int len_add,
+                    hipStream_t stream);
 void tl_prefill_attn(const void* q, const void* k, const void* v, void* out,
                      int B, int Sq, int Skv, int q_off, int Hq, int Hkv,
                      int D, float scale, int causal, hipStream_t stream);
-void tl_rope_append(const void* qkv, void* q_out, void* k_cache,
-                    void* v_cache, const void* positions,
+void tl_rope_append(const void* qkv, const void* bias, void* q_out,
+                    void* k_cache, void* v_cache, const void* positions,
                     const void* inv_freq, const void* block_table,
                     int64_t T, int row_stride, int S, int Hq, int Hkv,
-                    int D, int Smax, int bt_stride, hipStream_t stream);
+                    int D, int Smax, int bt_stride, int n_split,
+                    int inv_bf16, hipStream_t stream);
 void tl_swiglu_fused(const void* gu, void* out, int64_t N, int I,
                      hipStream_t stream);
 void tl_decode_attn_mfma(const void* q, const void* k_cache,
@@ -39,13 +44,20 @@
                          const void* block_table, void* out,
                          void* partial, void* partial_ml, int B, int Hq,
                          int Hkv, int Smax, int D, float scale, int n_split,
-                         int bt_stride, int per_row, hipStream_t stream);
+                         int bt_stride, int per_row, int len_add,
+                         hipStream_t stream);
 void tl_skinny_gemm(const void* x, const void* w, const void* bias,
                     void* out, void* partial, int M, int N, int K,
                     int n_split, hipStream_t stream);
 void tl_gemm_tiled(const void* x, const void* w, const void* bias, void* out,
                    void* partial, int M, int N, int K, int n_split,
                    hipStream_t stream);
+void tl_skinny_gemm_partials(const void* x, const void* w, const void* bias,
+                             void* out, void* partial, int M, int N, int K,
+                             int n_split, hipStream_t stream);
+void tl_gemm_tiled_partials(const void* x, const void* w, const void* bias,
+                            void* out, void* partial, int M, int N, int K,
+                            int n_split, hipStream_t stream);
 void tl_sample(const void* logits, const void* temps, const void* top_ps,
                const void* top_ks, const void* pres, const void* freqs,
                void* counts, const void* seeds, const void* ctr, void* out,
@@ -120,6 +132,46 @@
   return outs;
 }
 
+std::vector<Tensor> rmsnorm_add_fwd(Tensor x, Tensor residual,
+                                    c10::optional<Tensor> w, double eps,
+                                    int64_t mode) {
+  CHECK_IN(residual, torch::kBFloat16);
+  TORCH_CHECK(mode >= 1 && mode <= 3, "mode must be 1, 2 or 3");
+  const int H = residual.size(-1);
+  TORCH_CHECK(H % 8 == 0, "H must be divisible by 8");
+  TORCH_CHECK(H <= 16384, "rmsnorm supports H <= 16384");
+  const int64_t N = residual.numel() / H;
+  int n_split = 0;
+  if (x.scalar_type() == torch::kFloat) {
+    CHECK_IN(x, torch::kFloat);
+    TORCH_CHECK(x.dim() >= 2 && x.size(-1) == H &&
+                    x.numel() == x.size(0) * residual.numel(),
+                "partials must be [n_split, rows, H]");
+    n_split = (int)x.size(0);
+  } else {
+    CHECK_IN(x, torch::kBFloat16);
+    TORCH_CHECK(x.numel() == residual.numel() && x.size(-1) == H,
+                "x / residual shape mismatch");
+  }
+  auto r_out = torch::empty_like(residual);
+  Tensor y;
+  const void* wp = nullptr;
+  void* yp = nullptr;
+  if (mode != 3) {
+    TORCH_CHECK(w.has_value(), "weight required");
+    CHECK_IN(w.value(), torch::kBFloat16);
+    TORCH_CHECK(w->numel() == H, "weight size mismatch");
+    y = torch::empty_like(residual);
+    wp = w->data_ptr();
+    yp = y.data_ptr();
+  }
+  tl_rmsnorm_add_fwd(x.data_ptr(), residual.data_ptr(), wp, yp,
+                     r_out.data_ptr(), N, H, (float)eps, n_split, (int)mode,
+                     cur_stream());
+  if (mode == 3) return {r_out};
+  return {y, r_out};
+}
+
 std::vector<Tensor> rmsnorm_bwd(Tensor dy, Tensor x, Tensor w, Tensor rstd) {
   CHECK_IN(dy, torch::kBFloat16);
   CHECK_IN(x, torch::kBFloat16);
@@ -192,7 +244,7 @@
 
 Tensor decode_attn(Tensor q, Tensor k_cache, Tensor v_cache, Tensor seq_lens,
                    double scale, int64_t n_split,
-                   c10::optional<Tensor> block_table) {
+                   c10::optional<Tensor> block_table, int64_t len_add) {
   CHECK_IN(q, torch::kBFloat16);
   CHECK_IN(k_cache, torch::kBFloat16);
   CHECK_IN(v_cache, torch::kBFloat16);
@@ -217,7 +269,7 @@
   if (legacy) {
     tl_decode_attn(q.data_ptr(), k_cache.data_ptr(), v_cache.data_ptr(),
                    seq_lens.data_ptr(), out.data_ptr(), B, Hq, Hkv, Smax, D,
-                   (float)scale, cur_stream());
+                   (float)scale, (int)len_add, cur_stream());
     return out;
   }
   int per_row = 0;
@@ -240,7 +292,7 @@
   tl_decode_attn_mfma(q.data_ptr(), k_cache.data_ptr(), v_cache.data_ptr(),
                       seq_lens.data_ptr(), bt, out.data_ptr(), pp, pml, B,
                       Hq, Hkv, Smax, D, (float)scale, (int)n_split,
-                      bt_stride, per_row, cur_stream());
+                      bt_stride, per_row, (int)len_add, cur_stream());
   return out;
 }
 
@@ -304,16 +356,38 @@
 Tensor rope_append_(Tensor qkv, Tensor k_cache, Tensor v_cache,
                     Tensor positions, Tensor inv_freq, int64_t S,
                     int64_t Hq, int64_t Hkv,
-                    c10::optional<Tensor> block_table) {
-  CHECK_IN(qkv, torch::kBFloat16);
+                    c10::optional<Tensor> block_table,
+                    c10::optional<Tensor> bias) {
   CHECK_IN(k_cache, torch::kBFloat16);
   CHECK_IN(v_cache, torch::kBFloat16);
   CHECK_IN(positions, torch::kInt);
-  CHECK_IN(inv_freq, torch::kFloat);
+  TORCH_CHECK(inv_freq.is_cuda() && inv_freq.is_contiguous(),
+              "inv_freq must be a contiguous GPU tensor");
+  const bool inv_bf16 = inv_freq.scalar_type() == torch::kBFloat16;
+  TORCH_CHECK(inv_bf16 || inv_freq.scalar_type() == torch::kFloat,
+              "inv_freq must be fp32 or bf16");
   const int D = k_cache.size(3);
+  TORCH_CHECK(inv_freq.numel() >= D / 2, "inv_freq too short");
   const int row_stride = qkv.size(-1);
   TORCH_CHECK(row_stride == (Hq + 2 * Hkv) * D, "qkv width mismatch");
-  const int64_t T = qkv.numel() / row_stride;
+  int n_split = 0;
+  const void* bp = nullptr;
+  if (qkv.scalar_type() == torch::kFloat) {
+    CHECK_IN(qkv, torch::kFloat);
+    TORCH_CHECK(qkv.dim() >= 2, "partials must be [n_split, T, width]");
+    n_split = (int)qkv.size(0);
+    TORCH_CHECK(row_stride <= 32768, "qkv row too wide for the LDS stage");
+    if (bias.has_value()) {
+      CHECK_IN(bias.value(), torch::kBFloat16);
+      TORCH_CHECK(bias->numel() == row_stride, "bias size mismatch");
+      bp = bias->data_ptr();
+    }
+  } else {
+    CHECK_IN(qkv, torch::kBFloat16);
+    TORCH_CHECK(!bias.has_value(), "bias goes with partials only");
+  }
+  const int64_t T = qkv.numel() / row_stride / (n_split ? n_split : 1);
+  TORCH_CHECK(positions.numel() == T, "positions size mismatch");
   const int Smax = k_cache.size(2);
   TORCH_CHECK(T % S == 0, "T must be divisible by S");
   TORCH_CHECK(D % 16 == 0, "D must be divisible by 16");
@@ -328,11 +402,12 @@
   } else {
     TORCH_CHECK(k_cache.size(0) * S == T, "cache batch mismatch");
   }
-  auto q_out = torch::empty({T, Hq, (int64_t)D}, qkv.options());
-  tl_rope_append(qkv.data_ptr(), q_out.data_ptr(), k_cache.data_ptr(),
+  auto q_out = torch::empty({T, Hq, (int64_t)D}, k_cache.options());
+  tl_rope_append(qkv.data_ptr(), bp, q_out.data_ptr(), k_cache.data_ptr(),
                  v_cache.data_ptr(), positions.data_ptr(),
                  inv_freq.data_ptr(), bt, T, row_stride, (int)S, (int)Hq,
-                 (int)Hkv, D, Smax, bt_stride, cur_stream());
+                 (int)Hkv, D, Smax, bt_stride, n_split, inv_bf16 ? 1 : 0,
+                 cur_stream());
   return q_out;
 }
 
@@ -403,6 +478,31 @@
     tl_gemm_tiled(x.data_ptr(), w.data_ptr(), bp, out.data_ptr(), pp,
                   (int)M, N, K, n_split, cur_stream());
   return out;
+}
+
+Tensor skinny_gemm_partials(Tensor x, Tensor w, c10::optional<Tensor> bias) {
+  CHECK_IN(x, torch::kBFloat16);
+  CHECK_IN(w, torch::kBFloat16);
+  const int K = x.size(-1);
+  const int64_t M = x.numel() / K;
+  const int N = w.size(0);
+  TORCH_CHECK(w.size(1) == K, "K mismatch");
+  TORCH_CHECK(K % 32 == 0 && N % 64 == 0, "unsupported shape");
+  const int n_split = gemm_n_split(N, K);
+  if (n_split == 1) return skinny_gemm(x, w, bias);
+  auto sizes = x.sizes().vec();
+  sizes.back() = N;
+  sizes.insert(sizes.begin(), n_split);
+  auto partial = torch::empty(sizes, x.options().dtype(torch::kFloat));
+  if (M <= 64)
+    tl_skinny_gemm_partials(x.data_ptr(), w.data_ptr(), nullptr, nullptr,
+                            partial.data_ptr(), (int)M, N, K, n_split,
+                            cur_stream());
+  else
+    tl_gemm_tiled_partials(x.data_ptr(), w.data_ptr(), nullptr, nullptr,
+                           partial.data_ptr(), (int)M, N, K, n_split,
+                           cur_stream());
+  return partial;
 }
 
 static int mxfp4_split_for_blocks(int blocks, int K) {
@@ -611,6 +711,10 @@
           "fused RoPE + KV-cache append from fused-QKV rows");
   mod.def("swiglu_fused", &swiglu_fused, "silu-mul on fused [.,2I] rows");
   mod.def("skinny_gemm", &skinny_gemm, "decode-M GEMM: x @ W^T + bias");
+  mod.def("skinny_gemm_partials", &skinny_gemm_partials,
+          "decode-M GEMM handing out its fp32 split-K partials");
+  mod.def("rmsnorm_add_fwd", &rmsnorm_add_fwd,
+          "residual add + RMSNorm from bf16 or split-K partials");
   mod.def("rmsnorm_fwd", &rmsnorm_fwd, "fused RMSNorm fwd (+residual)");
   mod.def("rmsnorm_bwd", &rmsnorm_bwd, "RMSNorm bwd");
   mod.def("rope_", &rope_, "in-place RoPE apply");
diff --git a/tensorlink_amd/ops/csrc/common.hpp b/tensorlink_amd/ops/csrc/common.hpp
--- a/tensorlink_amd/ops/csrc/common.hpp
+++ b/tensorlink_amd/ops/csrc/common.hpp
@@ -68,6 +68,41 @@
   return (a + b - 1) / b;
 }
 
+template <int NV, int CH>
+DEVINLINE void sum_partials8(const float* (&p)[NV],
+                             int64_t split_stride, int n_split,
+                             float (&acc)[NV][8]) {
+#pragma unroll
+  for (int v = 0; v < NV; ++v)
+#pragma unroll
+    for (int j = 0; j < 8; ++j) acc[v][j] = 0.f;
+  for (int s0 = 0; s0 < n_split; s0 += CH) {
+    f32x4_u buf[NV][CH][2];
+#pragma unroll
+    for (int v = 0; v < NV; ++v)
+#pragma unroll
+      for (int k = 0; k < CH; ++k) {
+        const int s = min(s0 + k, n_split - 1);
+        const float4* q =
+            reinterpret_cast<const float4*>(p[v] + s * split_stride);
+        buf[v][k][0].f4 = q[0];
+        buf[v][k][1].f4 = q[1];
+      }
+#pragma unroll
+    for (int k = 0; k < CH; ++k) {
+      if (s0 + k < n_split) {
+#pragma unroll
+        for (int v = 0; v < NV; ++v)
+#pragma unroll
+          for (int j = 0; j < 4; ++j) {
+            acc[v][j] += buf[v][k][0].f[j];
+            acc[v][4 + j] += buf[v][k][1].f[j];
+          }
+      }
+    }
+  }
+}
+
 typedef __bf16 tr_bf16x8 __attribute__((ext_vector_type(8)));
 
 DEVINLINE tr_bf16x8 ds_read_tr16_frag(unsigned addr_bytes) {
diff --git a/tensorlink_amd/ops/csrc/decode_attn.hip b/tensorlink_amd/ops/csrc/decode_attn.hip
--- a/tensorlink_amd/ops/csrc/decode_attn.hip
+++ b/tensorlink_amd/ops/csrc/decode_attn.hip
@@ -15,7 +15,7 @@
     const bf16* __restrict__ v_cache,
     const int* __restrict__ seq_lens,
     bf16* __restrict__ out,
-    int Hq, int Hkv, int Smax, float scale) {
+    int Hq, int Hkv, int Smax, float scale, int len_add) {
   constexpr int EPL = D / LPK;
   const int b = blockIdx.x;
   const int hkv = blockIdx.y;
@@ -23,7 +23,7 @@
   const int g0 = blockIdx.z * GMAX;
   const int gq = min(GMAX, G - g0);
   const int h0 = hkv * G + g0;
-  const int L = seq_lens[b];
+  const int L = seq_lens[b] + len_add;
 
   const int lane = threadIdx.x & (WAVE_SIZE - 1);
   const int wave = threadIdx.x / WAVE_SIZE;
@@ -152,7 +152,8 @@
 
 void tl_decode_attn(const void* q, const void* k_cache, const void* v_cache,
                     const void* seq_lens, void* out, int B, int Hq, int Hkv,
-                    int Smax, int D, float scale, hipStream_t stream) {
+                    int Smax, int D, float scale, int len_add,
+                    hipStream_t stream) {
   const int G = Hq / Hkv;
   int gmax = G <= 2 ? 2 : 4;
   if (const char* e = getenv("TL_DECODE_GMAX")) gmax = atoi(e);
@@ -161,7 +162,7 @@
   hipLaunchKernelGGL((decode_attn_kernel<DD, GG>), grid, block, 0, stream, \
                      (const bf16*)q, (const bf16*)k_cache,                 \
                      (const bf16*)v_cache, (const int*)seq_lens,           \
-                     (bf16*)out, Hq, Hkv, Smax, scale)
+                     (bf16*)out, Hq, Hkv, Smax, scale, len_add)
   if (D == 128) {
     if (gmax == 2) LAUNCH(128, 2);
     else if (gmax == 4) LAUNCH(128, 4);
diff --git a/tensorlink_amd/ops/csrc/decode_attn_mfma.hip b/tensorlink_amd/ops/csrc/decode_attn_mfma.hip
--- a/tensorlink_amd/ops/csrc/decode_attn_mfma.hip
+++ b/tensorlink_amd/ops/csrc/decode_attn_mfma.hip
@@ -21,7 +21,7 @@
     float* __restrict__ partial,
     float* __restrict__ partial_ml,
     int Hq, int Hkv, int Smax, float scale, int n_split, int bt_stride,
-    int per_row) {
+    int per_row, int len_add) {
   constexpr int KCH = D / 32;
   constexpr int NS = D / 16;
   const int b = blockIdx.x;
@@ -29,7 +29,7 @@
   const int split = blockIdx.z;
   const int G = Hq / Hkv;
   const int h0 = hkv * G;
-  const int L = seq_lens[b];
+  const int L = seq_lens[b] + len_add;
 
   const int ns_row = per_row ? tl_split_for_len(L) : n_split;
   if (split >= ns_row) return;
@@ -211,11 +211,11 @@
 __global__ __launch_bounds__(128) void decode_attn_combine_kernel(
     const float* __restrict__ partial, const float* __restrict__ partial_ml,
     const int* __restrict__ seq_lens, bf16* __restrict__ out, int Hq,
-    int n_split, int per_row) {
+    int n_split, int per_row, int len_add) {
   const int bh = blockIdx.x;
   const int d = threadIdx.x;
   const int ns_row =
-      per_row ? tl_split_for_len(seq_lens[bh / Hq]) : n_split;
+      per_row ? tl_split_for_len(seq_lens[bh / Hq] + len_add) : n_split;
   __shared__ float sm[64], sl[64];
   if (threadIdx.x < ns_row) {
     sm[threadIdx.x] = partial_ml[((int64_t)bh * n_split + threadIdx.x) * 2];
@@ -242,7 +242,8 @@
                          const void* block_table, void* out,
                          void* partial, void* partial_ml, int B, int Hq,
                          int Hkv, int Smax, int D, float scale, int n_split,
-                         int bt_stride, int per_row, hipStream_t stream) {
+                         int bt_stride, int per_row, int len_add,
+                         hipStream_t stream) {
   dim3 grid(B, Hkv, n_split), block(BLOCK);
 #define LAUNCH(DD, SM, PG)                                                   \
   hipLaunchKernelGGL((decode_attn_mfma_kernel<DD, SM, PG>), grid, block, 0,  \
@@ -250,7 +251,7 @@
                      (const bf16*)v_cache, (const int*)seq_lens,             \
                      (const int*)block_table, (bf16*)out,                    \
                      (float*)partial, (float*)partial_ml, Hq, Hkv, Smax,     \
-                     scale, n_split, bt_stride, per_row)
+                     scale, n_split, bt_stride, per_row, len_add)
 #define PICK(DD)                                                             \
   do {                                                                       \
     if (block_table) {                                                       \
@@ -269,13 +270,13 @@
       hipLaunchKernelGGL((decode_attn_combine_kernel<128>), cgrid, cblock, 0,
                          stream, (const float*)partial,
                          (const float*)partial_ml, (const int*)seq_lens,
-                         (bf16*)out, Hq, n_split, per_row);
+                         (bf16*)out, Hq, n_split, per_row, len_add);
     else
       hipLaunchKernelGGL((decode_attn_combine_kernel<64>), cgrid, cblock, 0,
                          stream, (const float*)partial,
                          (const float*)partial_ml, (const int*)seq_lens,
-                         (bf16*)out, Hq, n_split, per_row);
-  }
-}
-
-}
+                         (bf16*)out, Hq, n_split, per_row, len_add);
+  }
+}
+
+}
diff --git a/tensorlink_amd/ops/csrc/gemm_tiled.hip b/tensorlink_amd/ops/csrc/gemm_tiled.hip
--- a/tensorlink_amd/ops/csrc/gemm_tiled.hip
+++ b/tensorlink_amd/ops/csrc/gemm_tiled.hip
@@ -270,13 +270,9 @@
   out[i] = f2bf(acc);
 }
 
-}
-
-extern "C" {
-
-void tl_gemm_tiled(const void* x, const void* w, const void* bias, void* out,
-                   void* partial, int M, int N, int K, int n_split,
-                   hipStream_t stream) {
+void tiled_launch(const void* x, const void* w, const void* bias, void* out,
+                  void* partial, int M, int N, int K, int n_split,
+                  int reduce, hipStream_t stream) {
   const int m_tiles = (M + 15) / 16;
   const int split = n_split > 1 ? 1 : 0;
   if (N >= 65536) {
@@ -315,7 +311,7 @@
   else DISPATCH(16);
 #undef DISPATCH
   }
-  if (split) {
+  if (split && reduce) {
     const int64_t MN = (int64_t)M * N;
     dim3 rgrid((uint32_t)((MN + 255) / 256)), rblock(256);
     if (bias)
@@ -330,3 +326,19 @@
 }
 
 }
+
+extern "C" {
+
+void tl_gemm_tiled(const void* x, const void* w, const void* bias, void* out,
+                   void* partial, int M, int N, int K, int n_split,
+                   hipStream_t stream) {
+  tiled_launch(x, w, bias, out, partial, M, N, K, n_split, 1, stream);
+}
+
+void tl_gemm_tiled_partials(const void* x, const void* w, const void* bias,
+                            void* out, void* partial, int M, int N, int K,
+                            int n_split, hipStream_t stream) {
+  tiled_launch(x, w, bias, out, partial, M, N, K, n_split, 0, stream);
+}
+
+}
diff --git a/tensorlink_amd/ops/csrc/rmsnorm.hip b/tensorlink_amd/ops/csrc/rmsnorm.hip
--- a/tensorlink_amd/ops/csrc/rmsnorm.hip
+++ b/tensorlink_amd/ops/csrc/rmsnorm.hip
@@ -6,15 +6,29 @@
 constexpr int BLOCK = 256;
 constexpr int NW = BLOCK / WAVE_SIZE;
 
-template <int ITERS, int RES>
+template <int ITERS, int RES, int PART>
 __global__ __launch_bounds__(BLOCK) void rmsnorm_fwd_kernel(
-    const bf16* __restrict__ x, const bf16* __restrict__ residual,
+    const void* __restrict__ x_, const bf16* __restrict__ residual,
     const bf16* __restrict__ w, bf16* __restrict__ y, bf16* __restrict__ r_out,
-    float* __restrict__ rstd_out, int H, float eps) {
+    float* __restrict__ rstd_out, int H, float eps, int n_split,
+    int64_t split_stride) {
   __shared__ float lds[NW];
   const int64_t row = blockIdx.x;
-  const bf16* xrow = x + row * H;
+  const bf16* xrow = PART ? nullptr : (const bf16*)x_ + row * H;
+  const float* prow = PART ? (const float*)x_ + row * H : nullptr;
   const bf16* rrow = RES ? residual + row * H : nullptr;
+
+  constexpr int CH = ITERS <= 2 ? 8 : ITERS <= 4 ? 4 : 2;
+  float psum[PART ? ITERS : 1][8];
+  if constexpr (PART) {
+    const float* pp[ITERS];
+#pragma unroll
+    for (int it = 0; it < ITERS; ++it) {
+      const int base = (it * BLOCK + threadIdx.x) * 8;
+      pp[it] = prow + (base < H ? base : 0);
+    }
+    sum_partials8<ITERS, CH>(pp, split_stride, n_split, psum);
+  }
 
   float vals[ITERS][8];
   float sumsq = 0.f;
@@ -22,18 +36,24 @@
   for (int it = 0; it < ITERS; ++it) {
     const int base = (it * BLOCK + threadIdx.x) * 8;
     if (base < H) {
-      bf16x8 vx = *reinterpret_cast<const bf16x8*>(xrow + base);
+      bf16x8 vx;
+      if constexpr (PART) {
+#pragma unroll
+        for (int j = 0; j < 8; ++j) vx.v[j] = f2bf(psum[it][j]);
+      } else {
+        vx = *reinterpret_cast<const bf16x8*>(xrow + base);
+      }
       if (RES) {
         bf16x8 vr = *reinterpret_cast<const bf16x8*>(rrow + base);
+        bf16x8 out;
 #pragma unroll
         for (int j = 0; j < 8; ++j) {
           float f = bf2f(vx.v[j]) + bf2f(vr.v[j]);
+          out.v[j] = f2bf(f);
+          if (RES >= 2) f = bf2f(out.v[j]);
           vals[it][j] = f;
           sumsq += f * f;
         }
-        bf16x8 out;
-#pragma unroll
-        for (int j = 0; j < 8; ++j) out.v[j] = f2bf(vals[it][j]);
         *reinterpret_cast<bf16x8*>(r_out + row * H + base) = out;
       } else {
 #pragma unroll
@@ -48,6 +68,7 @@
       for (int j = 0; j < 8; ++j) vals[it][j] = 0.f;
     }
   }
+  if (RES == 3) return;
 
   const float total = block_reduce_sum<NW>(sumsq, lds);
   const float rstd = rsqrtf(total / H + eps);
@@ -140,16 +161,18 @@
   out[i] = f2bf(acc);
 }
 
-template <int RES>
-void launch_fwd(const bf16* x, const bf16* res, const bf16* w, bf16* y,
+template <int RES, int PART>
+void launch_fwd(const void* x, const bf16* res, const bf16* w, bf16* y,
                 bf16* r_out, float* rstd, int64_t N, int H, float eps,
-                hipStream_t s) {
+                int n_split, hipStream_t s) {
   dim3 grid((uint32_t)N), block(BLOCK);
   const int iters = cdiv(H, BLOCK * 8);
-#define CASE(I)                                                            \
-  case I:                                                                  \
-    hipLaunchKernelGGL((rmsnorm_fwd_kernel<I, RES>), grid, block, 0, s, x, \
-                       res, w, y, r_out, rstd, H, eps);                    \
+  const int64_t split_stride = N * H;
+#define CASE(I)                                                              \
+  case I:                                                                    \
+    hipLaunchKernelGGL((rmsnorm_fwd_kernel<I, RES, PART>), grid, block, 0,   \
+                       s, x, res, w, y, r_out, rstd, H, eps, n_split,        \
+                       split_stride);                                        \
     break;
   switch (iters) {
     CASE(1) CASE(2) CASE(3) CASE(4) CASE(5) CASE(6) CASE(7) CASE(8)
@@ -166,11 +189,29 @@
                     void* y, void* r_out, void* rstd, int64_t N, int H,
                     float eps, hipStream_t stream) {
   if (residual)
-    launch_fwd<1>((const bf16*)x, (const bf16*)residual, (const bf16*)w,
-                  (bf16*)y, (bf16*)r_out, (float*)rstd, N, H, eps, stream);
+    launch_fwd<1, 0>(x, (const bf16*)residual, (const bf16*)w, (bf16*)y,
+                     (bf16*)r_out, (float*)rstd, N, H, eps, 1, stream);
   else
-    launch_fwd<0>((const bf16*)x, nullptr, (const bf16*)w, (bf16*)y, nullptr,
-                  (float*)rstd, N, H, eps, stream);
+    launch_fwd<0, 0>(x, nullptr, (const bf16*)w, (bf16*)y, nullptr,
+                     (float*)rstd, N, H, eps, 1, stream);
+}
+
+void tl_rmsnorm_add_fwd(const void* x, const void* residual, const void* w,
+                        void* y, void* r_out, int64_t N, int H, float eps,
+                        int n_split, int mode, hipStream_t stream) {
+#define GO(R, P)                                                          \
+  launch_fwd<R, P>(x, (const bf16*)residual, (const bf16*)w, (bf16*)y,    \
+                   (bf16*)r_out, nullptr, N, H, eps, n_split, stream)
+  if (n_split > 0) {
+    if (mode == 1) GO(1, 1);
+    else if (mode == 2) GO(2, 1);
+    else GO(3, 1);
+  } else {
+    if (mode == 1) GO(1, 0);
+    else if (mode == 2) GO(2, 0);
+    else GO(3, 0);
+  }
+#undef GO
 }
 
 void tl_rmsnorm_bwd(const void* dy, const void* x, const void* w,
diff --git a/tensorlink_amd/ops/csrc/rope_append.hip b/tensorlink_amd/ops/csrc/rope_append.hip
--- a/tensorlink_amd/ops/csrc/rope_append.hip
+++ b/tensorlink_amd/ops/csrc/rope_append.hip
@@ -5,13 +5,14 @@
 
 constexpr int BLOCK = 256;
 
-template <int PAGED>
+template <int PAGED, int PART>
 __global__ __launch_bounds__(BLOCK) void rope_append_kernel(
-    const bf16* __restrict__ qkv, bf16* __restrict__ q_out,
-    bf16* __restrict__ k_cache, bf16* __restrict__ v_cache,
-    const int* __restrict__ positions, const float* __restrict__ inv_freq,
-    const int* __restrict__ block_table, int row_stride, int S, int Hq,
-    int Hkv, int D, int Smax, int bt_stride) {
+    const void* __restrict__ qkv, const bf16* __restrict__ bias,
+    bf16* __restrict__ q_out, bf16* __restrict__ k_cache,
+    bf16* __restrict__ v_cache, const int* __restrict__ positions,
+    const void* __restrict__ inv_freq, const int* __restrict__ block_table,
+    int row_stride, int S, int Hq, int Hkv, int D, int Smax, int bt_stride,
+    int n_split, int64_t split_stride, int inv_bf16) {
   const int64_t token = blockIdx.x;
   const int b = token / S;
   const int pos = positions[token];
@@ -25,16 +26,60 @@
   const int64_t head_stride = PAGED ? 128 : Smax;
   const int D2 = D / 2;
   const float fpos = (float)pos;
-  const bf16* row = qkv + token * row_stride;
+  extern __shared__ __align__(16) unsigned char smem[];
+  const bf16* row;
+  if constexpr (PART) {
+    constexpr int UN = 3;
+    bf16* srow = reinterpret_cast<bf16*>(smem);
+    const float* prow = (const float*)qkv + token * row_stride;
+    const int n8 = row_stride / 8;
+    for (int g0 = 0; g0 < n8; g0 += BLOCK * UN) {
+      const float* pp[UN];
+#pragma unroll
+      for (int u = 0; u < UN; ++u)
+        pp[u] = prow + min(g0 + u * BLOCK + (int)threadIdx.x, n8 - 1) * 8;
+      float acc[UN][8];
+      sum_partials8<UN, 4>(pp, split_stride, n_split, acc);
+#pragma unroll
+      for (int u = 0; u < UN; ++u) {
+        const int g = g0 + u * BLOCK + threadIdx.x;
+        if (g < n8) {
+          bf16x8 out;
+          if (bias) {
+            const bf16x8 vb = *reinterpret_cast<const bf16x8*>(bias + g * 8);
+#pragma unroll
+            for (int j = 0; j < 8; ++j)
+              out.v[j] = f2bf(acc[u][j] + bf2f(vb.v[j]));
+          } else {
+#pragma unroll
+            for (int j = 0; j < 8; ++j) out.v[j] = f2bf(acc[u][j]);
+          }
+          reinterpret_cast<bf16x8*>(srow)[g] = out;
+        }
+      }
+    }
+    __syncthreads();
+    row = srow;
+  } else {
+    row = (const bf16*)qkv + token * row_stride;
+  }
   const bf16* krow = row + Hq * D;
   const bf16* vrow = krow + Hkv * D;
 
   const int total = (Hq + Hkv) * D2;
+  auto angle = [&](int d, float& s, float& c) {
+    const float fr = inv_bf16 ? bf2f(((const bf16*)inv_freq)[d])
+                              : ((const float*)inv_freq)[d];
+    __sincosf(fpos * fr, &s, &c);
+  };
+  const bool fixed_d = BLOCK % D2 == 0;
+  float c0 = 0.f, s0 = 0.f;
+  if (fixed_d) angle(threadIdx.x % D2, s0, c0);
   for (int idx = threadIdx.x; idx < total; idx += BLOCK) {
     const int h = idx / D2;
     const int d = idx - h * D2;
-    float c, s;
-    __sincosf(fpos * inv_freq[d], &s, &c);
+    float c = c0, s = s0;
+    if (!fixed_d) angle(d, s, c);
     if (h < Hq) {
       const bf16* src = row + h * D;
       const float x1 = bf2f(src[d]);
@@ -63,28 +108,49 @@
   }
 }
 
+template <int PART>
+void launch(const void* qkv, const void* bias, void* q_out, void* k_cache,
+            void* v_cache, const void* positions, const void* inv_freq,
+            const void* block_table, int64_t T, int row_stride, int S,
+            int Hq, int Hkv, int D, int Smax, int bt_stride, int n_split,
+            int inv_bf16, hipStream_t stream) {
+  dim3 grid((uint32_t)T), block(BLOCK);
+  const int64_t split_stride = T * row_stride;
+  const size_t lds = PART ? (size_t)row_stride * sizeof(bf16) : 0;
+  if (block_table)
+    hipLaunchKernelGGL((rope_append_kernel<1, PART>), grid, block, lds,
+                       stream, qkv, (const bf16*)bias, (bf16*)q_out,
+                       (bf16*)k_cache,
+                       (bf16*)v_cache, (const int*)positions, inv_freq,
+                       (const int*)block_table, row_stride, S, Hq, Hkv, D,
+                       Smax, bt_stride, n_split, split_stride, inv_bf16);
+  else
+    hipLaunchKernelGGL((rope_append_kernel<0, PART>), grid, block, lds,
+                       stream, qkv, (const bf16*)bias, (bf16*)q_out,
+                       (bf16*)k_cache,
+                       (bf16*)v_cache, (const int*)positions, inv_freq,
+                       nullptr, row_stride, S, Hq, Hkv, D, Smax, bt_stride,
+                       n_split, split_stride, inv_bf16);
+}
+
 }
 
 extern "C" {
 
-void tl_rope_append(const void* qkv, void* q_out, void* k_cache,
-                    void* v_cache, const void* positions,
+void tl_rope_append(const void* qkv, const void* bias, void* q_out,
+                    void* k_cache, void* v_cache, const void* positions,
                     const void* inv_freq, const void* block_table,
                     int64_t T, int row_stride, int S, int Hq, int Hkv,
-                    int D, int Smax, int bt_stride, hipStream_t stream) {
-  dim3 grid((uint32_t)T), block(BLOCK);
-  if (block_table)
-    hipLaunchKernelGGL((rope_append_kernel<1>), grid, block, 0, stream,
-                       (const bf16*)qkv, (bf16*)q_out, (bf16*)k_cache,
-                       (bf16*)v_cache, (const int*)positions,
-                       (const float*)inv_freq, (const int*)block_table,
-                       row_stride, S, Hq, Hkv, D, Smax, bt_stride);
+                    int D, int Smax, int bt_stride, int n_split,
+                    int inv_bf16, hipStream_t stream) {
+  if (n_split > 0)
+    launch<1>(qkv, bias, q_out, k_cache, v_cache, positions, inv_freq,
+              block_table, T, row_stride, S, Hq, Hkv, D, Smax, bt_stride,
+              n_split, inv_bf16, stream);
   else
-    hipLaunchKernelGGL((rope_append_kernel<0>), grid, block, 0, stream,
-                       (const bf16*)qkv, (bf16*)q_out, (bf16*)k_cache,
-                       (bf16*)v_cache, (const int*)positions,
-                       (const float*)inv_freq, nullptr, row_stride, S, Hq,
-                       Hkv, D, Smax, bt_stride);
+    launch<0>(qkv, nullptr, q_out, k_cache, v_cache, positions, inv_freq,
+              block_table, T, row_stride, S, Hq, Hkv, D, Smax, bt_stride, 0,
+              inv_bf16, stream);
 }
 
 }
diff --git a/tensorlink_amd/ops/csrc/skinny_gemm.hip b/tensorlink_amd/ops/csrc/skinny_gemm.hip
--- a/tensorlink_amd/ops/csrc/skinny_gemm.hip
+++ b/tensorlink_amd/ops/csrc/skinny_gemm.hip
@@ -111,13 +111,9 @@
   out[i] = f2bf(acc);
 }
 
-}
-
-extern "C" {
-
-void tl_skinny_gemm(const void* x, const void* w, const void* bias,
-                    void* out, void* partial, int M, int N, int K,
-                    int n_split, hipStream_t stream) {
+void skinny_launch(const void* x, const void* w, const void* bias,
+                   void* out, void* partial, int M, int N, int K,
+                   int n_split, int reduce, hipStream_t stream) {
   const int m_tiles = (M + 15) / 16;
   const int split = n_split > 1 ? 1 : 0;
   dim3 grid(N / 64, n_split), block(BLOCK);
@@ -144,7 +140,7 @@
   else if (m_tiles <= 8) DISPATCH(8);
   else DISPATCH(16);
 #undef DISPATCH
-  if (split) {
+  if (split && reduce) {
     const int64_t MN = (int64_t)M * N;
     dim3 rgrid((uint32_t)((MN + 255) / 256)), rblock(256);
     if (bias)
@@ -159,3 +155,19 @@
 }
 
 }
+
+extern "C" {
+
+void tl_skinny_gemm(const void* x, const void* w, const void* bias,
+                    void* out, void* partial, int M, int N, int K,
+                    int n_split, hipStream_t stream) {
+  skinny_launch(x, w, bias, out, partial, M, N, K, n_split, 1, stream);
+}
+
+void tl_skinny_gemm_partials(const void* x, const void* w, const void* bias,
+                             void* out, void* partial, int M, int N, int K,
+                             int n_split, hipStream_t stream) {
+  skinny_launch(x, w, bias, out, partial, M, N, K, n_split, 0, stream);
+}
+
+}
```

New measurement: 13680 tokens/s (median of 6 runs). 1.03x the previous value.
